# GSByeon/multi-speaker-tacotron-tensorflow

Measured on AMD Instinct MI355X. Metric: mel-frames/sec (batched decode), higher is better.
Workload: dtype f32 storage and accumulation; feed-forward GEMMs as 3-term split-bf16 MFMA (bf16x3), the attention memory layer as 6-term split-bf16 MFMA (operands split three ways: fp32-grade); recurrent / decoder mat-vecs exact fp32

## Files before the change

### include/taco_debug.h

```cpp
#ifndef TACO_DEBUG_H
#define TACO_DEBUG_H

#include "taco_abi.h"

#ifdef __cplusplus
extern "C" {
#endif

int taco_debug_set_persistent(taco_model* m, int on);

int taco_debug_set_bf3(taco_model* m, int on, int tile_n);

int taco_debug_set_fuse_prenet(taco_model* m, int on);
int taco_debug_set_fuse_concat(taco_model* m, int on);
int taco_debug_set_att_split(taco_model* m, int slices);
int taco_debug_set_overlap(taco_model* m, int on);

int taco_debug_set_decoder_persist(taco_model* m, int mode, int rows_per_group);
int taco_debug_raise_device_error(taco_model* m, int value);
int taco_debug_decoder_info(taco_model* m, int* out16);
int taco_debug_decoder_trace(taco_model* m, int enable, long long* out);

int taco_debug_set_skip_scans(taco_model* m, int on);

int taco_debug_set_chip_turns(int on);

int taco_debug_force_gemm_config(taco_model* m, int cfg);

int taco_debug_set_front(taco_model* m, int delay_clocks, int prio);

int taco_train_debug_bigru(taco_train* t, void* hip_stream, const float* d_xproj, const int32_t* d_lengths, const float* d_h0,
                           const float* d_dout, int B, int T, int persistent, float* d_out, float* d_gsave, float* d_dg, float* d_rh,
                           float* d_dh0, void* d_scratch, size_t scratch_bytes);

int taco_debug_wgrad_plan(int wgrad_bf3, int wgrad_planes, int deterministic, long long det_floats, long long planes_uint4, int region_open,
                          int M, int T, int K, int N, int kw, int padl, int gather, int ygather, int nw, int* out8);

int taco_debug_spec_epilogue(taco_gl* g, void* hip_stream, const float* d_est, int R, float* d_linear, float* d_mel);

int taco_debug_gl_create_host(const taco_audio_hparams* hp, int tf_flavor, taco_gl** out);

#ifdef __cplusplus
}
#endif
#endif
```

### multi-speaker-tacotron-tensorflow_amd/_lib.py

```python
import ctypes as C
import os

from .hparams import MODEL_TYPES, ATTENTION_TYPES, NUM_SYMBOLS

_HERE = os.path.dirname(os.path.abspath(__file__))
LIB_PATH = os.path.join(_HERE, "csrc", "libtaco_hip.so")

TACO_ERR_ARG, TACO_ERR_SHAPE, TACO_ERR_UNSUPPORTED, TACO_ERR_HIP, TACO_ERR_STATE = -1, -2, -3, -4, -5
TACO_TRIM_SPECTRAL, TACO_TRIM_TIME = 0, 1
TACO_WAV_F32, TACO_WAV_PCM16 = 0, 1


class TacoHParams(C.Structure):
    _fields_ = [
        ("num_symbols", C.c_int32), ("num_mels", C.c_int32), ("num_freq", C.c_int32),
        ("num_speakers", C.c_int32), ("model_type", C.c_int32), ("speaker_embedding_size", C.c_int32),
        ("embedding_size", C.c_int32),
        ("enc_prenet_n", C.c_int32), ("enc_prenet", C.c_int32 * 4),
        ("enc_bank_size", C.c_int32), ("enc_bank_channels", C.c_int32), ("enc_maxpool", C.c_int32),
        ("enc_highway_depth", C.c_int32), ("enc_rnn_size", C.c_int32),
        ("enc_proj_n", C.c_int32), ("enc_proj", C.c_int32 * 4), ("enc_proj_width", C.c_int32),
        ("attention_type", C.c_int32), ("attention_size", C.c_int32), ("attention_state_size", C.c_int32),
        ("dec_layer_num", C.c_int32), ("dec_rnn_size", C.c_int32),
        ("dec_prenet_n", C.c_int32), ("dec_prenet", C.c_int32 * 4),
# ... 13 lines not shown
class TacoCollateStream(C.Structure):
    _fields_ = [("pack", C.c_void_p), ("start", C.c_void_p), ("rows", C.c_void_p), ("width", C.c_int32), ("rows_out", C.c_int32),
                ("out", C.c_void_p), ("counts", C.c_void_p)]


TACO_COLLATE_MAX_STREAMS = 8


class TacoError(Exception):

    def __init__(self, code, msg):
        super().__init__(msg)
        self.code = code


def _list4(vals, what):
    vals = list(vals)
    if not 1 <= len(vals) <= 4:
        raise TacoError(TACO_ERR_ARG, "%s must have 1..4 entries, got %d" % (what, len(vals)))
    arr = (C.c_int32 * 4)(*(vals + [0] * (4 - len(vals))))
    return len(vals), arr


def to_c_hparams(hp, num_speakers):
    if hp.model_type not in MODEL_TYPES:
        raise Exception(" [!] Unkown multi-speaker model type: {}".format(hp.model_type))
    if hp.attention_type not in ATTENTION_TYPES:
        raise Exception(" [!] Unkown attention type: {}".format(hp.attention_type))
    c = TacoHParams()
    c.num_symbols = getattr(hp, "num_symbols", NUM_SYMBOLS)
    c.num_mels, c.num_freq = hp.num_mels, hp.num_freq
    c.num_speakers = int(num_speakers)
    c.model_type = MODEL_TYPES[hp.model_type]
    c.speaker_embedding_size = hp.speaker_embedding_size
    c.embedding_size = hp.embedding_size
    c.enc_prenet_n, c.enc_prenet = _list4(hp.enc_prenet_sizes, "enc_prenet_sizes")
    c.enc_bank_size, c.enc_bank_channels = hp.enc_bank_size, hp.enc_bank_channel_size
    c.enc_maxpool, c.enc_highway_depth, c.enc_rnn_size = hp.enc_maxpool_width, hp.enc_highway_depth, hp.enc_rnn_size
    c.enc_proj_n, c.enc_proj = _list4(hp.enc_proj_sizes, "enc_proj_sizes")
    c.enc_proj_width = hp.enc_proj_width
    c.attention_type = ATTENTION_TYPES[hp.attention_type]
    c.attention_size, c.attention_state_size = hp.attention_size, hp.attention_state_size
    c.dec_layer_num, c.dec_rnn_size = hp.dec_layer_num, hp.dec_rnn_size
    c.dec_prenet_n, c.dec_prenet = _list4(hp.dec_prenet_sizes, "dec_prenet_sizes")
    c.post_bank_size, c.post_bank_channels = hp.post_bank_size, hp.post_bank_channel_size
    c.post_maxpool, c.post_highway_depth, c.post_rnn_size = hp.post_maxpool_width, hp.post_highway_depth, hp.post_rnn_size
    c.post_proj_n, c.post_proj = _list4(hp.post_proj_sizes, "post_proj_sizes")
    c.post_proj_width = hp.post_proj_width
    c.reduction_factor, c.max_iters = hp.reduction_factor, hp.max_iters
    return c


_P = C.c_void_p
_I = C.c_int
_S = C.c_size_t
SYNC_SUM_FN = C.CFUNCTYPE(None, C.c_void_p, C.c_void_p, C.c_int)

PROTOTYPES = {
    "taco_abi_version": (_I, []),
    "taco_last_error": (C.c_char_p, []),
    "taco_model_create": (_I, [C.POINTER(TacoHParams), _I, C.POINTER(_P)]),
    "taco_model_set_weight": (_I, [_P, C.c_char_p, _P, C.POINTER(C.c_int64), _I]),
    "taco_model_num_weights": (_I, [_P]),
    "taco_model_weight_name": (_I, [_P, _I, C.c_char_p, _I, C.POINTER(C.c_int64), C.POINTER(_I)]),
    "taco_model_finalize": (_I, [_P]),
    "taco_model_destroy": (None, [_P]),
    "taco_workspace_bytes": (_S, [_P, _I, _I, _I]),
    "taco_stage_workspace_bytes": (_S, [_P, _I, _I]),
    "taco_forward_infer": (_I, [_P, _P, _P, _P, _P, _I, _I, _I, _P, _P, _P, _P, _P, _P, _S]),
    "taco_plan_create": (_I, [_P, _P, _P, _P, _I, _I, _I, _P, _P, _P, _P, _P, _P, _S, C.POINTER(_P)]),
    "taco_plan_launch": (_I, [_P, _P]),
    "taco_plan_num_nodes": (_I, [_P]),
    "taco_plan_whole_chip": (_I, [_P]),
    "taco_plan_destroy": (None, [_P]),
    "taco_encoder_forward": (_I, [_P, _P, _P, _P, _P, _I, _I, _P, _P, _S]),
    "taco_decoder_forward": (_I, [_P, _P, _P, _P, _I, _I, _I, _P, _P, _P, _P, _P, _P, _P, _S]),
    "taco_postnet_forward": (_I, [_P, _P, _P, _P, _I, _I, _P, _P, _P, _S]),
    "taco_conv1d_bn_f32": (_I, [_P, _P, C.c_char_p, _P, _I, _I, _I, _I, _P]),
    "taco_dense_f32": (_I, [_P, _P, C.c_char_p, _P, _I, _I, _P]),
    "taco_highway_f32": (_I, [_P, _P, C.c_char_p, _P, _I, _P]),
    "taco_bigru_f32": (_I, [_P, _P, C.c_char_p, _P, _P, _P, _I, _I, _P, _P, _S]),
    "taco_attention_step_f32": (_I, [_P, _P, _P, _P, _P, _P, _I, _I, _P, _P, _P, _S]),
    "taco_gru_cell_f32": (_I, [_P, _P, C.c_char_p, _P, _P, _I, _P, _P, _S]),
    "taco_gl_create": (_I, [C.POINTER(TacoAudioHParams), _I, C.POINTER(_P)]),
    "taco_gl_destroy": (None, [_P]),
    "taco_gl_num_samples": (_I, [_P, _I]),
    "taco_gl_workspace_bytes": (_S, [_P, _I, _I]),
    "taco_gl_inv_spectrogram": (_I, [_P, _P, _P, _P, C.c_ulonglong, _I, _I, _I, _P, _P, _S]),
    "taco_gl_min_frames": (_I, [_P]),
    "taco_gl_rows_workspace_bytes": (_S, [_P, _I, _I]),
    "taco_gl_inv_spectrogram_rows": (_I, [_P, _P, _P, _P, _P, C.c_ulonglong, _I, _I, _I, _P, _P, _P, _S]),
    "taco_wav_to_pcm16": (_I, [_P, _P, _P, _I, _I, _P]),
    "taco_gl_create_tf": (_I, [C.POINTER(TacoAudioHParams), _I, C.POINTER(_P)]),
    "taco_gl_tf_num_samples": (_I, [_P, _I]),
    "taco_gl_tf_workspace_bytes": (_S, [_P, _I, _I]),
    "taco_gl_inv_spectrogram_tf": (_I, [_P, _P, _P, _P, _I, _I, _I, _P, _P, _P, _S]),
    "taco_gl_set_inv_mel_basis": (_I, [_P, _P, _I]),
    "taco_gl_mel_to_linear": (_I, [_P, _P, _P, _I, _I, _P]),
    "taco_gl_inv_melspectrogram_rows": (_I, [_P, _P, _P, _P, _P, C.c_ulonglong, _I, _I, _I, _P, _P, _P, _S]),
    "taco_debug_gl_create_host": (_I, [C.POINTER(TacoAudioHParams), _I, C.POINTER(_P)]),
    "taco_wav_trim_workspace_bytes": (_S, [_I, _I, _I, _I]),
    "taco_wav_trim": (_I, [_P, _P, _P, _I, _I, C.c_float, _I, _I, _I, _P, _P, _P, _S]),
    "taco_wav_split_workspace_bytes": (_S, [_I, _I, _I, _I]),
    "taco_wav_split": (_I, [_P, _P, _P, _I, _I, C.c_float, _I, _I, _I, _I, _P, _P, _P, _P, _S]),
    "taco_wav_breath_mute": (_I, [_P, _P, _P, _I, _I, _P, _P, _I, C.c_float, _P, _P, _P]),
    "taco_resample_create": (_I, [_I, _I, _P, _I, _I, _I, C.POINTER(_P)]),
    "taco_resample_destroy": (None, [_P]),
    "taco_resample_out_len": (_I, [_P, _I]),
    "taco_resample_computed_len": (_I, [_P, _I]),
    "taco_resample_phases": (_I, [_P]),
    "taco_resample_taps": (_I, [_P]),
    "taco_resample_left_taps": (_I, [_P]),
    "taco_resample_tile": (_I, [_P]),
    "taco_resample_bank": (_I, [_P, _P]),
    "taco_wav_resample": (_I, [_P, _P, _P, _I, _I, _P, _I, _I, _P, _I, _P]),
    "taco_gl_set_mel_basis": (_I, [_P, _P, _I]),
    "taco_spec_num_mels": (_I, [_P]),
    "taco_spec_num_frames": (_I, [C.POINTER(TacoAudioHParams), _I]),
    "taco_spec_workspace_bytes": (_S, [_P, _I, _I]),
    "taco_spec_targets": (_I, [_P, _P, _P, _P, _I, _I, _P, _P, _P, _P, _S]),
    "taco_collate": (_I, [_P, C.POINTER(TacoCollateStream), _I, _P, _I, _I]),
    "taco_debug_spec_epilogue": (_I, [_P, _P, _P, _I, _P, _P]),
    "taco_attention_trim": (_I, [_P, _P, _P, _I, _I, _I, _I, _P]),
    "taco_loss_f32": (_I, [_P, _P, _P, _P, _P, _P, _I, _I, _I, _I, _I, _I, _P, _P, _S]),
    "taco_learning_rate": (C.c_float, [C.c_longlong, C.c_float, _I, _I]),
    "taco_adam_step_f32": (_I, [_P, _P, _P, _P, _P, _S, C.c_longlong, C.c_float, C.c_float, C.c_float, C.c_float, C.c_float, _P, _P, _S]),
    "taco_train_create": (_I, [C.POINTER(TacoHParams), _I, C.POINTER(_P)]),
    "taco_train_destroy": (None, [_P]),
    "taco_train_model": (_P, [_P]),
    "taco_train_num_params": (_S, [_P]),
    "taco_train_param_offset": (_I, [_P, C.c_char_p, C.POINTER(_S)]),
    "taco_train_refresh": (_I, [_P, _P, _P]),
    "taco_train_set_sync_bn": (_I, [_P, _P, _P, _I]),
    "taco_train_set_deterministic": (_I, [_P, _I]),
    "taco_train_set_exact_wgrad": (_I, [_P, _I]),
    "taco_train_set_wgrad_planes": (_I, [_P, _I]),
    "taco_train_planes_problems": (_I, [_P]),
    "taco_train_set_bptt_engine": (_I, [_P, _I]),
    "taco_train_set_exact_gemm": (_I, [_P, _I]),
    "taco_debug_wgrad_plan": (_I, [_I, _I, _I, C.c_longlong, C.c_longlong, _I, _I, _I, _I, _I, _I, _I, _I, _I, _I, C.POINTER(_I)]),
    "taco_train_debug_bigru": (_I, [_P, _P, _P, _P, _P, _P, _I, _I, _I, _P, _P, _P, _P, _P, _P, _S]),
    "taco_train_workspace_bytes": (_S, [_P, _I, _I, _I]),
    "taco_train_forward_backward": (_I, [_P, _P, _P, _P, _P, _P, _P, _P, _P, _P, _I, _I, _I, _I, _I, _P, _P, _P, _P, _I, _P, _S]),
    "taco_debug_force_gemm_config": (_I, [_P, _I]),
    "taco_debug_set_skip_scans": (_I, [_P, _I]),
    "taco_debug_set_chip_turns": (_I, [_I]),
    "taco_debug_set_front": (_I, [_P, _I, _I]),
    "taco_debug_set_persistent": (_I, [_P, _I]),
    "taco_debug_set_overlap": (_I, [_P, _I]),
    "taco_stop_steps": (_I, [_P, _P, _I, _I, _I, _I, _P]),
    "taco_debug_set_fuse_prenet": (_I, [_P, _I]),
    "taco_debug_set_fuse_concat": (_I, [_P, _I]),
    "taco_debug_set_att_split": (_I, [_P, _I]),
    "taco_debug_set_bf3": (_I, [_P, _I, _I]),
    "taco_model_device_errors": (_I, [_P, C.POINTER(_I)]),
    "taco_debug_raise_device_error": (_I, [_P, _I]),
    "taco_debug_set_decoder_persist": (_I, [_P, _I, _I]),
    "taco_debug_decoder_info": (_I, [_P, C.POINTER(_I)]),
    "taco_model_engine_plan": (_I, [_P, _I, _I, _I, _I, C.c_char_p, _I]),
    "taco_model_set_batch_invariant": (_I, [_P, _I]),
    "taco_debug_decoder_trace": (_I, [_P, _I, C.POINTER(C.c_longlong)]),
}

_lib = None


def load_library(path=None):
    global _lib
    if _lib is not None and path is None:
        return _lib
    p = path or os.environ.get("TACO_LIB") or LIB_PATH
    if path is None and os.environ.get("TACO_LIB") and os.path.abspath(p) != os.path.abspath(LIB_PATH):
        import warnings
        warnings.warn("TACO_LIB overrides the library: loading %s instead of %s" % (p, LIB_PATH), RuntimeWarning, stacklevel=2)
    if not os.path.exists(p):
        raise ImportError(
            "libtaco_hip.so not found at %s -- build it first (python -c 'import __graft_entry__ as g; g.build()' "
            "or multi-speaker-tacotron-tensorflow_amd/csrc/build.sh).  There is no CPU fallback." % p)
    lib = C.CDLL(p)
    for name, (res, args) in PROTOTYPES.items():
        fn = getattr(lib, name)
        fn.restype = res
        fn.argtypes = args
    if lib.taco_abi_version() != 1:
        raise ImportError("libtaco_hip.so ABI version %d, expected 1" % lib.taco_abi_version())
    if path is None:
        _lib = lib
    return lib


def check(rc):
    if rc != 0:
        msg = load_library().taco_last_error().decode("utf-8", "replace")
        if rc == TACO_ERR_UNSUPPORTED and msg.startswith(" [!]"):
            raise Exception(msg)
        raise TacoError(rc, "libtaco_hip error %d: %s" % (rc, msg))
```

### multi-speaker-tacotron-tensorflow_amd/csrc/taco_chain.h

```cpp
#pragma once
#include "taco_kernels.h"

#define CH_MAXL 8
#ifndef CH_PF256
#define CH_PF256 2
#endif
#ifndef CH_PF128
#define CH_PF128 2
#endif
#ifndef CH_ROT
#define CH_ROT 1
#endif
#define CH_BM 64
enum { CH_DENSE = 0, CH_HIGHWAY = 1, CH_XPROJ = 2 };
struct ChainLayer {
  const unsigned short* bh; const unsigned short* bl; const unsigned short* bh2; const unsigned short* bl2;
  const float* bias; const float* bias2;
  int type, K16, NT, N, act;
};
struct ChainEntry {
  const float* part; int P; size_t MN; int N1;
  const float* b1; const float* s1; const float* h1; int relu1;
  const unsigned short* bh; const unsigned short* bl; int NT2, K16tap, N2;
  const float* b2; const float* s2; const float* h2;
  const float* res; int ldres;
  const float* rowvec; int ldrv;
};
struct ChainArgs {
  ChainEntry e;
  const float* x; int ldx, Cin;
  const int* gather;
  float* out; int ldo;
  float* y; int ldy;
  const int* rev_len; int rev_col0;
  int M, T, nlayers;
  int krot;
  int ntiles; unsigned* zp[4]; unsigned long long znw[4];
  ChainLayer L[CH_MAXL];
};

template <int TM, int LDSW, bool DUAL, int CH_PF>
__device__ __forceinline__ void ch_mma_loop(int K16, int NT, const unsigned short* bhA, const unsigned short* blA, int nt,
                                            const unsigned short* bhB, const unsigned short* blB, int nt2,
                                            const unsigned short* xhi, const unsigned short* xlo, int row0,
                                            int l31, int lh, f32x16 (&acc)[TM], f32x16 (&acc2)[TM], int rot = 0) {
  auto kstep = [&](int g) { const int gg = min(g, K16 - 1) + rot; return gg >= K16 ? gg - K16 : gg; };
  auto boff = [&](int g, int t) { return ((((size_t)kstep(g) * NT + t) * 2 + lh) * 32 + l31) * 8; };
  uint4 ph, pl, ph2, pl2, qh, ql, qh2, ql2;
  ph2 = pl2 = qh2 = ql2 = make_uint4(0, 0, 0, 0);
  auto loadb = [&](int g, uint4& h, uint4& l, uint4& h2, uint4& l2) {
    const size_t o = boff(g, nt);
    h = *reinterpret_cast<const uint4*>(bhA + o); l = *reinterpret_cast<const uint4*>(blA + o);
    if constexpr (DUAL) { const size_t o2 = boff(g, nt2); h2 = *reinterpret_cast<const uint4*>(bhB + o2); l2 = *reinterpret_cast<const uint4*>(blB + o2); }
  };
  auto mma = [&](int g, const uint4& h, const uint4& l, const uint4& h2, const uint4& l2) {
    const bf16x8 bh = __builtin_bit_cast(bf16x8, h), bl = __builtin_bit_cast(bf16x8, l);
    bf16x8 ah[TM], al[TM];
#pragma unroll
    for (int tm = 0; tm < TM; ++tm) {
      const int off = (row0 + tm * 32 + l31) * LDSW + 16 * kstep(g) + 8 * lh;
      ah[tm] = __builtin_bit_cast(bf16x8, *reinterpret_cast<const uint4*>(xhi + off));
      al[tm] = __builtin_bit_cast(bf16x8, *reinterpret_cast<const uint4*>(xlo + off));
    }
#pragma unroll
    for (int tm = 0; tm < TM; ++tm) acc[tm] = __builtin_amdgcn_mfma_f32_32x32x16_bf16(al[tm], bh, acc[tm], 0, 0, 0);
#pragma unroll
    for (int tm = 0; tm < TM; ++tm) acc[tm] = __builtin_amdgcn_mfma_f32_32x32x16_bf16(ah[tm], bl, acc[tm], 0, 0, 0);
#pragma unroll
    for (int tm = 0; tm < TM; ++tm) acc[tm] = __builtin_amdgcn_mfma_f32_32x32x16_bf16(ah[tm], bh, acc[tm], 0, 0, 0);
    if constexpr (DUAL) {
      const bf16x8 bh2 = __builtin_bit_cast(bf16x8, h2), bl2 = __builtin_bit_cast(bf16x8, l2);
#pragma unroll
      for (int tm = 0; tm < TM; ++tm) acc2[tm] = __builtin_amdgcn_mfma_f32_32x32x16_bf16(al[tm], bh2, acc2[tm], 0, 0, 0);
#pragma unroll
      for (int tm = 0; tm < TM; ++tm) acc2[tm] = __builtin_amdgcn_mfma_f32_32x32x16_bf16(ah[tm], bl2, acc2[tm], 0, 0, 0);
#pragma unroll
      for (int tm = 0; tm < TM; ++tm) acc2[tm] = __builtin_amdgcn_mfma_f32_32x32x16_bf16(ah[tm], bh2, acc2[tm], 0, 0, 0);
    }
  };
  if constexpr (CH_PF == 2) {
  loadb(0, ph, pl, ph2, pl2);
  for (int g = 0; g < K16; g += 2) {
    loadb(g + 1, qh, ql, qh2, ql2);
    __builtin_amdgcn_sched_barrier(0);
    mma(g, ph, pl, ph2, pl2);
    __builtin_amdgcn_sched_barrier(0);
    loadb(g + 2, ph, pl, ph2, pl2);
    __builtin_amdgcn_sched_barrier(0);
    mma(g + 1, qh, ql, qh2, ql2);
    __builtin_amdgcn_sched_barrier(0);
  }
  } else {
  uint4 rh[CH_PF], rl[CH_PF], rh2[CH_PF], rl2[CH_PF];
#pragma unroll
  for (int i = 0; i < CH_PF; ++i) rh2[i] = rl2[i] = make_uint4(0, 0, 0, 0);
#pragma unroll
  for (int i = 0; i < CH_PF - 1; ++i) loadb(i, rh[i], rl[i], rh2[i], rl2[i]);
  for (int g = 0; g < K16; g += CH_PF) {
#pragma unroll
    for (int i = 0; i < CH_PF; ++i) {
      loadb(g + i + CH_PF - 1, rh[(i + CH_PF - 1) % CH_PF], rl[(i + CH_PF - 1) % CH_PF], rh2[(i + CH_PF - 1) % CH_PF], rl2[(i + CH_PF - 1) % CH_PF]);
      __builtin_amdgcn_sched_barrier(0);
      if (g + i < K16) mma(g + i, rh[i], rl[i], rh2[i], rl2[i]);
      __builtin_amdgcn_sched_barrier(0);
    }
  }
  }
}

#ifdef TACO_TRACE
__device__ long long taco_trace_chain[64];
#define CTRC(i) do { if (trc && (i) < 64) taco_trace_chain[i] = clock64(); } while (0)
#else
#define CTRC(i) do {} while (0)
#endif
template <int W>
__global__ __launch_bounds__(512) void k_pointwise_chain(const ChainArgs a_in) {
  constexpr int WN = W / 32, WM = 8 / WN, TM = CH_BM / 32 / WM;
  constexpr int PF = W == 256 ? CH_PF256 : CH_PF128;
  constexpr int LDSW = W + 8;
  extern __shared__ __attribute__((aligned(16))) unsigned short ch_smem[];
  unsigned short* xhi = ch_smem;
  unsigned short* xlo = ch_smem + CH_BM * LDSW;
  struct { const float* x; float* out; float* y; const int* rev_len; int ldx, Cin, ldo, ldy, rev_col0, M, T, nlayers; } a =
      {a_in.x, a_in.out, a_in.y, a_in.rev_len, a_in.ldx, a_in.Cin, a_in.ldo, a_in.ldy, a_in.rev_col0, a_in.M, a_in.T, a_in.nlayers};
  PIN(a.x); PIN(a.out); PIN(a.y); PIN(a.rev_len); PIN(a.ldx); PIN(a.Cin); PIN(a.ldo); PIN(a.ldy); PIN(a.rev_col0); PIN(a.M); PIN(a.T);
  PIN(a.nlayers);
  const int tid = threadIdx.x, lane = tid & 63, l31 = lane & 31, lh = lane >> 5;
  const int wave = __builtin_amdgcn_readfirstlane(tid >> 6);
  const int wm = wave / WN, wn = wave % WN;
  if (a_in.ntiles > 0 && (int)blockIdx.x >= a_in.ntiles) {
    const size_t i0 = (size_t)((int)blockIdx.x - a_in.ntiles) * 512 + tid, stride = (size_t)((int)gridDim.x - a_in.ntiles) * 512;
    for (int rg = 0; rg < 4; ++rg) {
      unsigned* p = a_in.zp[rg];
      const size_t nw = a_in.znw[rg];
      if (!p || !nw) continue;
      const size_t n16 = (reinterpret_cast<uintptr_t>(p) & 15) ? 0 : nw / 4;
      uint4* q = reinterpret_cast<uint4*>(p);
      for (size_t i = i0; i < n16; i += stride) q[i] = make_uint4(0u, 0u, 0u, 0u);
      for (size_t i = n16 * 4 + i0; i < nw; i += stride) p[i] = 0u;
    }
    return;
  }
  const int m0 = blockIdx.x * CH_BM;
  const int krot = (CH_ROT && a_in.krot) ? ((int)(blockIdx.x >> 3) & 31) : 0;
#ifdef TACO_TRACE
  const bool trc = (blockIdx.x == (a_in.ntiles > 0 ? a_in.ntiles : gridDim.x) / 2) && threadIdx.x == 0;
  int trci = 5;
  CTRC(0);
#endif

  const int l31_outer = l31, lh_outer = lh;
  float xreg[TM][16];
  bool have_x = false;
  if (a_in.e.part) {
    const ChainEntry E = a_in.e;
    const float* gpart = E.part; const float* gb1 = E.b1; const float* gs1 = E.s1; const float* gh1 = E.h1;
    const unsigned short* gbh = E.bh; const unsigned short* gbl = E.bl;
    const float* gres = E.res; const float* grv = E.rowvec; const float* gb2 = E.b2; const float* gs2 = E.s2; const float* gh2 = E.h2;
    PIN(gpart); PIN(gb1); PIN(gs1); PIN(gh1); PIN(gbh); PIN(gbl); PIN(gres); PIN(grv); PIN(gb2); PIN(gs2); PIN(gh2);
    const int LDE = E.N1 + 8;
    unsigned short* ehi = ch_smem + 2 * CH_BM * LDSW;
    unsigned short* elo = ehi + (CH_BM + 2) * LDE;
    const int nq = E.N1 / 4;
    constexpr int NSTG = ((CH_BM + 2) * (256 / 4) + 511) / 512;
    {
      float4 f[NSTG];
      const float* src[NSTG];
#pragma unroll
      for (int u = 0; u < NSTG; ++u) {
        const int i = tid + 512 * u, r = i / nq, c = 4 * (i - r * nq), row = m0 - 1 + r;
        f[u] = make_float4(0.f, 0.f, 0.f, 0.f);
        src[u] = (i < (CH_BM + 2) * nq && row >= 0 && row < a.M) ? gpart + (size_t)row * E.N1 + c : nullptr;
      }
      int q = 0;
      for (; q + 1 < E.P; q += 2) {
        float4 g[NSTG], g2[NSTG];
#pragma unroll
        for (int u = 0; u < NSTG; ++u) {
          g[u] = src[u] ? *reinterpret_cast<const float4*>(src[u] + (size_t)q * E.MN) : make_float4(0.f, 0.f, 0.f, 0.f);
          g2[u] = src[u] ? *reinterpret_cast<const float4*>(src[u] + (size_t)(q + 1) * E.MN) : make_float4(0.f, 0.f, 0.f, 0.f);
        }
#pragma unroll
        for (int u = 0; u < NSTG; ++u) { f[u].x += g[u].x; f[u].y += g[u].y; f[u].z += g[u].z; f[u].w += g[u].w; }
#pragma unroll
        for (int u = 0; u < NSTG; ++u) { f[u].x += g2[u].x; f[u].y += g2[u].y; f[u].z += g2[u].z; f[u].w += g2[u].w; }
      }
      if (q < E.P) {
        float4 g[NSTG];
#pragma unroll
        for (int u = 0; u < NSTG; ++u) g[u] = src[u] ? *reinterpret_cast<const float4*>(src[u] + (size_t)q * E.MN) : make_float4(0.f, 0.f, 0.f, 0.f);
#pragma unroll
        for (int u = 0; u < NSTG; ++u) { f[u].x += g[u].x; f[u].y += g[u].y; f[u].z += g[u].z; f[u].w += g[u].w; }
      }
#pragma unroll
      for (int u = 0; u < NSTG; ++u) {
        const int i = tid + 512 * u, r = i / nq, c = 4 * (i - r * nq);
        if (i >= (CH_BM + 2) * nq) continue;
        float4 v = f[u];
        if (src[u]) {
          const float4 bi = gb1 ? *reinterpret_cast<const float4*>(gb1 + c) : make_float4(0.f, 0.f, 0.f, 0.f);
          const float4 sc = gs1 ? *reinterpret_cast<const float4*>(gs1 + c) : make_float4(1.f, 1.f, 1.f, 1.f);
          const float4 sh = gh1 ? *reinterpret_cast<const float4*>(gh1 + c) : make_float4(0.f, 0.f, 0.f, 0.f);
          v.x += bi.x; v.y += bi.y; v.z += bi.z; v.w += bi.w;
          if (E.relu1) { v.x = fmaxf(v.x, 0.f); v.y = fmaxf(v.y, 0.f); v.z = fmaxf(v.z, 0.f); v.w = fmaxf(v.w, 0.f); }
          v.x = v.x * sc.x + sh.x; v.y = v.y * sc.y + sh.y; v.z = v.z * sc.z + sh.z; v.w = v.w * sc.w + sh.w;
        }
        uint2 h4, l4;
        taco_split_bf16x4(v, h4, l4);
        *reinterpret_cast<uint2*>(ehi + r * LDE + c) = h4;
        *reinterpret_cast<uint2*>(elo + r * LDE + c) = l4;
      }
    }
    CTRC(1);
    __syncthreads();
    const int K0 = a_in.L[0].K16 * 16;
    const int col = wn * 32 + l31;
    const bool cin = col < E.N2;
    float rs[TM][16];
#pragma unroll
    for (int tm = 0; tm < TM; ++tm)
#pragma unroll
      for (int r = 0; r < 16; ++r) {
        const int rl = (wm * TM + tm) * 32 + (r & 3) + 8 * (r >> 2) + 4 * lh, row = min(m0 + rl, a.M - 1);
        float v = 0.f;
        if (cin) {
          v = gres[(size_t)row * E.ldres + col];
          if (grv) v += grv[(size_t)(row / a.T) * E.ldrv + col];
        }
        rs[tm][r] = v;
      }
    f32x16 acc[TM];
#pragma unroll
    for (int tm = 0; tm < TM; ++tm)
      for (int r = 0; r < 16; ++r) acc[tm][r] = 0.f;
    const int KSPL = (WM == 1 && 2 * E.NT2 <= WN) ? 2 : 1;
    const bool mact = wn < E.NT2 * KSPL;
    const int ect = mact ? wn % E.NT2 : 0, kp = mact ? wn / E.NT2 : 0;
    if (mact) {
      int tloc[TM];
#pragma unroll
      for (int tm = 0; tm < TM; ++tm) tloc[tm] = (m0 + (wm * TM + tm) * 32 + l31) % a.T;
      const int nk = (3 * E.K16tap) / KSPL, kbeg = kp * nk, kend = kbeg + nk;
      auto boff = [&](int k) { return ((((size_t)k * E.NT2 + ect) * 2 + lh) * 32 + l31) * 8; };
      constexpr int NB = 6;
      uint4 pH[NB], pL[NB], qH[NB], qL[NB];
      auto loadblk = [&](int k0, uint4 (&H)[NB], uint4 (&Lo)[NB]) {
#pragma unroll
        for (int i = 0; i < NB; ++i) { const size_t o = boff(min(k0 + i, kend - 1)); H[i] = *reinterpret_cast<const uint4*>(gbh + o); Lo[i] = *reinterpret_cast<const uint4*>(gbl + o); }
      };
      auto mmablk = [&](int k0, const uint4 (&H)[NB], const uint4 (&Lo)[NB]) {
#pragma unroll
        for (int i = 0; i < NB; ++i) {
          const int k = k0 + i, j = k / E.K16tap, g = k - j * E.K16tap;
          const bf16x8 bh8 = __builtin_bit_cast(bf16x8, H[i]), bl8 = __builtin_bit_cast(bf16x8, Lo[i]);
#pragma unroll
          for (int tm = 0; tm < TM; ++tm) {
            const int off = ((wm * TM + tm) * 32 + l31 + j) * LDE + 16 * g + 8 * lh;
            uint4 xh = *reinterpret_cast<const uint4*>(ehi + off), xl = *reinterpret_cast<const uint4*>(elo + off);
            const int tt = tloc[tm] + j - 1;
            const unsigned keep = ((tt >= 0) && (tt < a.T)) ? 0xffffffffu : 0u;
            xh.x &= keep; xh.y &= keep; xh.z &= keep; xh.w &= keep; xl.x &= keep; xl.y &= keep; xl.z &= keep; xl.w &= keep;
            const bf16x8 ah = __builtin_bit_cast(bf16x8, xh), al = __builtin_bit_cast(bf16x8, xl);
            acc[tm] = __builtin_amdgcn_mfma_f32_32x32x16_bf16(al, bh8, acc[tm], 0, 0, 0);
            acc[tm] = __builtin_amdgcn_mfma_f32_32x32x16_bf16(ah, bl8, acc[tm], 0, 0, 0);
            acc[tm] = __builtin_amdgcn_mfma_f32_32x32x16_bf16(ah, bh8, acc[tm], 0, 0, 0);
          }
        }
      };
      loadblk(kbeg, pH, pL);
      for (int k0 = kbeg; k0 < kend; k0 += 2 * NB) {
        loadblk(k0 + NB, qH, qL);
        __builtin_amdgcn_sched_barrier(0);
        mmablk(k0, pH, pL);
        __builtin_amdgcn_sched_barrier(0);
        loadblk(k0 + 2 * NB, pH, pL);
        __builtin_amdgcn_sched_barrier(0);
        mmablk(k0 + NB, qH, qL);
        __builtin_amdgcn_sched_barrier(0);
      }
    }
    if (KSPL == 2) {
      float* red = reinterpret_cast<float*>(ch_smem);
      if (mact && kp == 1) {
#pragma unroll
        for (int tm = 0; tm < TM; ++tm)
#pragma unroll
          for (int r = 0; r < 16; ++r) red[((ect * TM + tm) * 16 + r) * 64 + lane] = acc[tm][r];
      }
      __syncthreads();
      if (mact && kp == 0) {
#pragma unroll
        for (int tm = 0; tm < TM; ++tm)
#pragma unroll
          for (int r = 0; r < 16; ++r) acc[tm][r] += red[((ect * TM + tm) * 16 + r) * 64 + lane];
      } else {
#pragma unroll
        for (int tm = 0; tm < TM; ++tm)
          for (int r = 0; r < 16; ++r) acc[tm][r] = 0.f;
      }
      __syncthreads();
    }
    CTRC(2);
    {
      const float bi = (cin && gb2) ? gb2[col] : 0.f, sc = (cin && gs2) ? gs2[col] : 1.f, sh = (cin && gh2) ? gh2[col] : 0.f;
#pragma unroll
      for (int tm = 0; tm < TM; ++tm)
#pragma unroll
        for (int r = 0; r < 16; ++r) asm volatile("" : "+v"(rs[tm][r]));
#pragma unroll
      for (int tm = 0; tm < TM; ++tm)
#pragma unroll
        for (int r = 0; r < 16; ++r) {
          const int rl = (wm * TM + tm) * 32 + (r & 3) + 8 * (r >> 2) + 4 * lh;
          const float v = cin ? (acc[tm][r] + bi) * sc + sh + rs[tm][r] : 0.f;
          xreg[tm][r] = v;
          if (col < K0) {
            const unsigned hp = taco_pk_bf16(v, 0.f) & 0xffffu;
            const unsigned lp = taco_pk_bf16(v - __uint_as_float(hp << 16), 0.f) & 0xffffu;
            xhi[rl * LDSW + col] = (unsigned short)hp;
            xlo[rl * LDSW + col] = (unsigned short)lp;
          }
        }
      have_x = true;
    }
    CTRC(3);
  } else
  {
    const int K0 = a_in.L[0].K16 * 16;
    for (int i = tid; i < CH_BM * (K0 / 4); i += 512) {
      const int r = i / (K0 / 4), c = 4 * (i % (K0 / 4));
      float4 f = make_float4(0.f, 0.f, 0.f, 0.f);
      const int row = m0 + r;
      if (row < a.M && c < a.Cin) {
        const float* p = a.x + (size_t)(a_in.gather ? a_in.gather[row] : row) * a.ldx + c;
        if (c + 3 < a.Cin && (a.ldx & 3) == 0) f = *reinterpret_cast<const float4*>(p);
        else { f.x = p[0]; if (c + 1 < a.Cin) f.y = p[1]; if (c + 2 < a.Cin) f.z = p[2]; if (c + 3 < a.Cin) f.w = p[3]; }
      }
      uint2 h4, l4;
      taco_split_bf16x4(f, h4, l4);
      *reinterpret_cast<uint2*>(xhi + r * LDSW + c) = h4;
      *reinterpret_cast<uint2*>(xlo + r * LDSW + c) = l4;
    }
  }
  const bool full = m0 + CH_BM <= a.M;
  __syncthreads();
  CTRC(4);

  for (int li = 0; li < a.nlayers; ++li) {
    const ChainLayer L = a_in.L[li];
    int l31 = l31_outer, lh = lh_outer;
    asm volatile("" : "+v"(l31), "+v"(lh));
    auto rloc = [&](int tm, int r) { return (wm * TM + tm) * 32 + (r & 3) + 8 * (r >> 2) + 4 * lh; };
    const int col = wn * 32 + l31;
    if (L.type == CH_XPROJ) {
      const int ngroups = (L.N + W - 1) / W;
      const int bb0 = m0 / a.T;
      const int nbrow = (a.M - 1) / a.T;
      const int Lb0 = a.rev_len ? a.rev_len[min(bb0, nbrow)] : a.T, Lb1 = a.rev_len ? a.rev_len[min(bb0 + 1, nbrow)] : a.T;
      auto store_group = [&](int ng, const f32x16 (&acc)[TM]) {
        const int ocol = ng * W + col;
        if (ocol >= L.N) return;
        const float bia = L.bias ? L.bias[ocol] : 0.f;
        const bool rev = a.rev_col0 >= 0 && ocol >= a.rev_col0;
        const bool relu_out = L.act == ACT_RELU;
        if (full && !rev) {
#pragma unroll
          for (int tm = 0; tm < TM; ++tm) {
            float* po = a.out + (size_t)(m0 + rloc(tm, 0)) * a.ldo + ocol;
#pragma unroll
            for (int r = 0; r < 16; ++r) { const float v = acc[tm][r] + bia; po[(size_t)((r & 3) + 8 * (r >> 2)) * a.ldo] = relu_out ? fmaxf(v, 0.f) : v; }
          }
        } else {
          int lhs = lh;
          asm volatile("" : "+v"(lhs));
#pragma unroll
          for (int tm = 0; tm < TM; ++tm)
#pragma unroll
            for (int r = 0; r < 16; ++r) {
              const int row = m0 + (wm * TM + tm) * 32 + (r & 3) + 8 * (r >> 2) + 4 * lhs;
              int orow = row;
              if (rev) {
                const int bb = a.T >= CH_BM ? bb0 + (row >= (bb0 + 1) * a.T ? 1 : 0) : row / a.T;
                const int tt = row - bb * a.T, Lb = a.T >= CH_BM ? (bb == bb0 ? Lb0 : Lb1) : (a.rev_len ? a.rev_len[min(bb, (a.M - 1) / a.T)] : a.T);
                orow = tt < Lb ? bb * a.T + (Lb - 1 - tt) : row;
              }
              if (row < a.M) { const float v = acc[tm][r] + bia; a.out[(size_t)orow * a.ldo + ocol] = relu_out ? fmaxf(v, 0.f) : v; }
            }
        }
      };
      const int npass = (ngroups + 1) / 2, odd = ngroups & 1;
      for (int ps = 0; ps < npass; ++ps) {
        const int ng = (odd && ps == 0) ? ngroups - 1 : 2 * (ps - odd);
        const int nt = min(ng * WN + wn, L.NT - 1), nt2 = min((ng + 1) * WN + wn, L.NT - 1);
        f32x16 acc[TM], acc2[TM];
#pragma unroll
        for (int tm = 0; tm < TM; ++tm)
          for (int r = 0; r < 16; ++r) { acc[tm][r] = 0.f; acc2[tm][r] = 0.f; }
        if (ng + 1 < ngroups) ch_mma_loop<TM, LDSW, true, PF>(L.K16, L.NT, L.bh, L.bl, nt, L.bh, L.bl, nt2, xhi, xlo, wm * TM * 32, l31, lh, acc, acc2, krot * L.K16 >> 5);
        else ch_mma_loop<TM, LDSW, false, PF>(L.K16, L.NT, L.bh, L.bl, nt, L.bh, L.bl, nt, xhi, xlo, wm * TM * 32, l31, lh, acc, acc2, krot * L.K16 >> 5);
#ifdef TACO_TRACE
        CTRC(trci); ++trci;
#endif
        store_group(ng, acc);
        if (ng + 1 < ngroups) store_group(ng + 1, acc2);
#ifdef TACO_TRACE
        CTRC(trci); ++trci;
#endif
      }
      continue;
    }
    const bool dual = L.type == CH_HIGHWAY;
    if (dual && !have_x) {
#pragma unroll
      for (int tm = 0; tm < TM; ++tm)
#pragma unroll
        for (int r = 0; r < 16; ++r) xreg[tm][r] = a.x[(size_t)min(m0 + rloc(tm, r), a.M - 1) * a.ldx + col];
    }
    have_x = true;
    {
      f32x16 acc[TM], acc2[TM];
#pragma unroll
      for (int tm = 0; tm < TM; ++tm)
        for (int r = 0; r < 16; ++r) { acc[tm][r] = 0.f; acc2[tm][r] = 0.f; }
      const float bia = L.bias ? L.bias[col] : 0.f;
      if (dual) {
        const float bia2 = L.bias2 ? L.bias2[col] : 0.f;
        ch_mma_loop<TM, LDSW, true, PF>(L.K16, L.NT, L.bh, L.bl, wn, L.bh2, L.bl2, wn, xhi, xlo, wm * TM * 32, l31, lh, acc, acc2, krot * L.K16 >> 5);
#ifdef TACO_TRACE
        CTRC(trci); ++trci;
#endif
#pragma unroll
        for (int tm = 0; tm < TM; ++tm)
#pragma unroll
          for (int r = 0; r < 16; ++r) {
            const float Hh = fmaxf(acc[tm][r] + bia, 0.f);
            const float Tg = __builtin_amdgcn_rcpf(1.0f + __builtin_amdgcn_exp2f(-1.4426950408889634f * (acc2[tm][r] + bia2)));
            xreg[tm][r] = Hh * Tg + xreg[tm][r] * (1.f - Tg);
          }
      } else {
        ch_mma_loop<TM, LDSW, false, PF>(L.K16, L.NT, L.bh, L.bl, wn, L.bh, L.bl, wn, xhi, xlo, wm * TM * 32, l31, lh, acc, acc2, krot * L.K16 >> 5);
#ifdef TACO_TRACE
        CTRC(trci); ++trci;
#endif
        const bool relu = L.act == ACT_RELU;
#pragma unroll
        for (int tm = 0; tm < TM; ++tm)
#pragma unroll
          for (int r = 0; r < 16; ++r) { const float v = acc[tm][r] + bia; xreg[tm][r] = relu ? fmaxf(v, 0.f) : v; }
      }
    }
    const bool last_hidden = (li + 1 == a.nlayers) || a_in.L[li + 1].type == CH_XPROJ;
    if (last_hidden && a.y) {
#pragma unroll
      for (int tm = 0; tm < TM; ++tm)
#pragma unroll
        for (int r = 0; r < 16; ++r) {
          const int row = m0 + rloc(tm, r);
          if (row < a.M) a.y[(size_t)row * a.ldy + col] = xreg[tm][r];
        }
    }
#ifdef TACO_TRACE
    CTRC(trci); ++trci;
#endif
    __syncthreads();
#ifdef TACO_TRACE
    CTRC(trci); ++trci;
#endif
#pragma unroll
    for (int tm = 0; tm < TM; ++tm)
#pragma unroll
      for (int r = 0; r < 16; ++r) {
        const float f = xreg[tm][r];
        const unsigned hp = taco_pk_bf16(f, 0.f) & 0xffffu;
        const unsigned lp = taco_pk_bf16(f - __uint_as_float(hp << 16), 0.f) & 0xffffu;
        xhi[rloc(tm, r) * LDSW + col] = (unsigned short)hp;
        xlo[rloc(tm, r) * LDSW + col] = (unsigned short)lp;
      }
    __syncthreads();
#ifdef TACO_TRACE
    CTRC(trci); ++trci;
#endif
  }
}
```

### multi-speaker-tacotron-tensorflow_amd/csrc/taco_lib.hip

```cpp
#include "taco_kernels.h"
#include "taco_decoder_xcd.h"
#include "taco_bigru_xcd.h"
#include "taco_chain.h"
#include "taco_front.h"
#include "taco_head.h"
#include "taco_train_kernels.h"
#include "taco_backward_kernels.h"
#include "taco_wgrad_planes.h"
#include "taco_decoder_bwd_xcd.h"
#include "../../include/taco_abi.h"
#include "../../include/taco_debug.h"

#include <algorithm>
#include <cmath>
#include <cstdarg>
#include <cstdio>
#include <cstring>
#include <cstdlib>
#include <functional>
#include <map>
#include <string>
#include <vector>

static thread_local std::string g_err;
// ... 42 lines not shown
  for (size_t i = n16 * 4 + i0; i < nw; i += stride) p[i] = 0u;
}
struct ZeroRegions { uint32_t* p[4]; unsigned long long nw[4]; };
__global__ void k_zero_fill_multi(const ZeroRegions z) {
  uint32_t* p = z.p[blockIdx.y];
  const size_t nw = z.nw[blockIdx.y];
  const size_t n16 = (reinterpret_cast<uintptr_t>(p) & 15) ? 0 : nw / 4;
  const size_t i0 = (size_t)blockIdx.x * blockDim.x + threadIdx.x, stride = (size_t)gridDim.x * blockDim.x;
  uint4* q = reinterpret_cast<uint4*>(p);
  for (size_t i = i0; i < n16; i += stride) q[i] = make_uint4(0u, 0u, 0u, 0u);
  for (size_t i = n16 * 4 + i0; i < nw; i += stride) p[i] = 0u;
}
#define ZM_MAX 12
struct ZeroMany { uint32_t* p[ZM_MAX]; unsigned long long nw[ZM_MAX]; };
__global__ void k_zero_fill_many(const ZeroMany z) {
  uint32_t* p = z.p[blockIdx.y];
  const size_t nw = z.nw[blockIdx.y];
  const size_t n16 = (reinterpret_cast<uintptr_t>(p) & 15) ? 0 : nw / 4;
  const size_t i0 = (size_t)blockIdx.x * blockDim.x + threadIdx.x, stride = (size_t)gridDim.x * blockDim.x;
  uint4* q = reinterpret_cast<uint4*>(p);
  for (size_t i = i0; i < n16; i += stride) q[i] = make_uint4(0u, 0u, 0u, 0u);
  for (size_t i = n16 * 4 + i0; i < nw; i += stride) p[i] = 0u;
}
struct ClearedSet { const void* p[8]; size_t n[8]; int cnt; };
static thread_local ClearedSet g_cleared = {};
static void register_cleared(const ZeroRegions& z) {
  for (int i = 0; i < 4; ++i)
    if (z.p[i] && g_cleared.cnt < 8) { g_cleared.p[g_cleared.cnt] = z.p[i]; g_cleared.n[g_cleared.cnt++] = z.nw[i] * 4; }
}
static hipError_t zero_async(void* p, size_t bytes, hipStream_t st);
static hipError_t clear_polled(void* p, size_t bytes, hipStream_t st) {
  for (int i = 0; i < g_cleared.cnt; ++i)
    if (g_cleared.p[i] == p && g_cleared.n[i] >= bytes) return hipSuccess;
  return zero_async(p, bytes, st);
}
static hipError_t zero_async(void* p, size_t bytes, hipStream_t st) {
  if (!bytes) return hipSuccess;
  if ((reinterpret_cast<uintptr_t>(p) & 3) || (bytes & 3)) return hipMemsetAsync(p, 0, bytes, st);
  const size_t nw = bytes / 4;
  const size_t n16 = (reinterpret_cast<uintptr_t>(p) & 15) ? 0 : nw / 4;
  const size_t items = n16 ? n16 + (nw - n16 * 4) : nw;
  const unsigned blocks = (unsigned)std::min<size_t>((items + 255) / 256, 2048);
  hipLaunchKernelGGL(k_zero_fill, dim3(blocks), dim3(256), 0, st, static_cast<uint32_t*>(p), n16, nw);
  return hipGetLastError();
}

struct ZeroBatch {
  ZeroMany z; int n = 0; size_t big = 0; hipStream_t st;
  explicit ZeroBatch(hipStream_t s) : st(s) { memset(&z, 0, sizeof z); }
  hipError_t add(void* p, size_t bytes) {
    if (!bytes) return hipSuccess;
    if ((reinterpret_cast<uintptr_t>(p) & 3) || (bytes & 3)) return zero_async(p, bytes, st);
    if (n == ZM_MAX) { hipError_t e = run(); if (e != hipSuccess) return e; }
    z.p[n] = static_cast<uint32_t*>(p); z.nw[n] = bytes / 4; big = std::max(big, bytes / 16); ++n;
    return hipSuccess;
  }
  hipError_t run() {
    if (!n) return hipSuccess;
    const unsigned blocks = (unsigned)std::min<size_t>(std::max<size_t>((big + 255) / 256, 1), 1024);
    hipLaunchKernelGGL(k_zero_fill_many, dim3(blocks, n), dim3(256), 0, st, z);
    n = 0; big = 0; memset(&z, 0, sizeof z);
    return hipGetLastError();
  }
};

#define HIPCHK(expr)                                                                        \
  do {                                                                                      \
    hipError_t e_ = (expr);                                                                 \
    if (e_ != hipSuccess) return fail(TACO_ERR_HIP, "%s: %s", #expr, hipGetErrorString(e_)); \
  } while (0)
#define TRY(expr)            \
  do {                       \
    int rc_ = (expr);        \
    if (rc_ != 0) return rc_; \
  } while (0)

static inline int cdiv(int a, int b) { return (a + b - 1) / b; }
static inline int rup(int a, int b) { return cdiv(a, b) * b; }
static inline size_t rup_sz(size_t a, size_t b) { return (a + b - 1) / b * b; }

struct HostTensor {
  std::vector<int64_t> shape;
  std::vector<float> data;
  bool set = false;
};

struct ConvL {
  int kw = 1, cin = 0, cin_pad = 0, N = 0;
  size_t wp = 0, wp2 = 0, bias = 0, bias2 = 0, bns = 0, bnb = 0;
  size_t bh = 0, bl = 0, bh2 = 0, bl2 = 0;
  size_t bl3 = 0, bl3_2 = 0;
  bool x6 = false;
  int K16 = 0, cin_pad16 = 0;
  size_t wtail = 0; int ntail = 0;
  int var_index = -1;
};
struct SkW {
  int K = 0, Kq = 0, N = 0;
  size_t wp = 0, bias = 0;
};
struct GruDec { SkW gx, ch; int I = 0, H = 0; };
struct Cbhg {
  int in_dim = 0, K = 0, C = 0, maxpool = 1, depth = 0, rnn = 0, pw = 3;
  int nproj = 0, proj_dim[4] = {0, 0, 0, 0};
  std::vector<ConvL> bank;
  int bank_var0 = -1;
  std::vector<ConvL> proj;
  bool has_dense = false;
  ConvL dense;
  std::vector<ConvL> hw;
  ConvL xproj;
  SkW gh[2], ch[2];
  size_t raw_gh[2] = {0, 0}, raw_ch[2] = {0, 0};
  size_t res_g2[2] = {0, 0};
  size_t gd_pack = 0, gb_pack = 0;
  size_t gob_pack = 0;
  size_t go_pack[3] = {0, 0, 0};
  std::vector<size_t> fr_wh, fr_wl; std::vector<int> fr_ns; int front_kind = 0;
  size_t res_g2p[2] = {0, 0}, res_c1p[2] = {0, 0};
};

struct taco_model {
  taco_hparams hp;
  int device = 0;
  bool finalized = false;
  std::vector<std::pair<std::string, std::vector<int64_t>>> spec;
  std::map<std::string, HostTensor> raw;
  std::vector<float> harena;
  float* darena = nullptr;
  size_t arena_n = 0;
  std::vector<GemmVar> hvars;
  std::map<std::string, ConvL> convs;
  std::map<std::string, SkW> skinny;
  std::map<std::string, GruDec> grus;
  std::vector<ConvL> enc_prenet;
  Cbhg enc, post;
  ConvL memory_layer, linear;
  std::vector<SkW> dec_prenet;
  GruDec att_gru;
  std::vector<GruDec> dec_gru;
  SkW query, concat_proj, frame_proj, lin_spk;
  SkW prenet1_next;
  int fuse_prenet1 = 1;
  GruDec gru1_fold;
  int fuse_concat = 0;
  int att_split = -1;
  size_t att_v = 0, att_b = 0, att_sb = 0, emb = 0, spk_emb = 0, raw_wq = 0;
  std::vector<SkW> spk_dense;
  std::vector<size_t> spk_table;
  int force_cfg = -1;
  unsigned* d_err = nullptr;
  int persist = 1;
  int ff_rot = 1;
  int bf3 = 1;
  int bf3x6 = 0;
  int bf3_tn = 0;
  int chain = 1;
  int front_entry = 1;
  int front_prio = 1; int front_delay = 0;
  int head_sweep = 1;
  int front = 1;
  int overlap = 0;
  size_t dx_fold_n = 0;
  size_t dx_spkw = 0;
  std::vector<unsigned> bf3_idx; std::vector<Bf3Seg> bf3_segs;
  int last_bptt = 0;
  size_t dbx_pack = 0;
  size_t dx_pack = 0, dx_p1o_raw = 0, dx_qpack[4] = {0, 0, 0, 0}, dx_b_p1_0 = 0, dx_b_p1c = 0, dx_b_p2 = 0, dx_b_p3 = 0, dx_b_ag = 0, dx_b_ac = 0, dx_b_g1f = 0,
         dx_b_g1c = 0, dx_b_g2g = 0, dx_b_g2c = 0, dx_b_f = 0;
  int cu_count = 0;
  int dx_mode = 1;
  int dx_rows = 0;
  long long* d_trace = nullptr;
  int trace_on = 0;
  int skip_scans = 0;
  hipStream_t side = nullptr;
  std::vector<hipEvent_t> events;
  struct TrainPacks* tp = nullptr;
};
static int build_train_packs(taco_model* m);

static size_t arena_put(taco_model* m, const float* src, size_t n) {
  size_t off = rup_sz(m->harena.size(), 16);
  m->harena.resize(off + rup_sz(std::max<size_t>(n, 1), 16), 0.f);
  if (src) memcpy(&m->harena[off], src, n * sizeof(float));
  return off + 1;
}
static inline const float* AP(const taco_model* m, size_t off1) { return off1 ? m->darena + (off1 - 1) : nullptr; }

static void spec_add(taco_model* m, const std::string& n, std::vector<int64_t> s) { m->spec.push_back({n, s}); }
static void spec_dense(taco_model* m, const std::string& n, int i, int o, bool bias = true) {
  spec_add(m, n + "/kernel", {i, o});
  if (bias) spec_add(m, n + "/bias", {o});
}
static void spec_conv(taco_model* m, const std::string& n, int k, int i, int o) {
  spec_add(m, n + "/kernel", {k, i, o});
  spec_add(m, n + "/bias", {o});
  for (const char* p : {"gamma", "beta", "moving_mean", "moving_variance"}) spec_add(m, n + "/" + p, {o});
}
static void spec_gru(taco_model* m, const std::string& n, int i, int h) {
  spec_add(m, n + "/gates/kernel", {i + h, 2 * h});
  spec_add(m, n + "/gates/bias", {2 * h});
  spec_add(m, n + "/candidate/kernel", {i + h, h});
  spec_add(m, n + "/candidate/bias", {h});
}
static void spec_cbhg(taco_model* m, const std::string& sc, int in_dim, int K, int C, int depth, int rnn,
                      const int* projs, int nproj, int pw) {
  for (int k = 1; k <= K; ++k) spec_conv(m, sc + "/conv_bank/conv1d_" + std::to_string(k), k, in_dim, C);
  int d = K * C;
  for (int i = 0; i < nproj; ++i) {
    spec_conv(m, sc + "/proj_" + std::to_string(i + 1), pw, d, projs[i]);
    d = projs[i];
  }
  if (d != rnn) spec_dense(m, sc + "/dense", d, rnn);
  for (int i = 0; i < depth; ++i) {
    spec_dense(m, sc + "/highway_" + std::to_string(i + 1) + "/H", rnn, rnn);
    spec_dense(m, sc + "/highway_" + std::to_string(i + 1) + "/T", rnn, rnn);
  }
  spec_gru(m, sc + "/bigru/fw", rnn, rnn);
  spec_gru(m, sc + "/bigru/bw", rnn, rnn);
}
static const char* kSpkNames[3] = {"before_highway", "encoder_rnn_init", "attention_rnn_init"};

static int build_spec(taco_model* m) {
  const taco_hparams& hp = m->hp;
  m->spec.clear();
  spec_add(m, "embedding", {hp.num_symbols, hp.embedding_size});
  const bool multi = hp.num_speakers > 1;
  const int spk = hp.speaker_embedding_size;
  if (multi) {
    if (spk != 1) spec_add(m, "speaker_embedding", {hp.num_speakers, spk});
    if (hp.model_type == 2) {
      std::vector<std::pair<std::string, int>> dims = {{kSpkNames[0], hp.enc_prenet[hp.enc_prenet_n - 1]},
                                                       {kSpkNames[1], hp.enc_rnn_size * 2},
                                                       {kSpkNames[2], hp.attention_state_size}};
      for (int i = 0; i < hp.dec_layer_num; ++i) dims.push_back({"decoder_rnn_init_" + std::to_string(i + 1), hp.dec_rnn_size});
      for (auto& d : dims) {
        if (spk == 1) spec_add(m, "spk/" + d.first + "/table", {hp.num_speakers, d.second});
        else spec_dense(m, "spk/" + d.first, spk, d.second);
      }
    }
  }
  int d = hp.embedding_size;
  for (int i = 0; i < hp.enc_prenet_n; ++i) {
    spec_dense(m, "prenet/dense_" + std::to_string(i + 1), d, hp.enc_prenet[i]);
    d = hp.enc_prenet[i];
  }
  spec_cbhg(m, "encoder_cbhg", d, hp.enc_bank_size, hp.enc_bank_channels, hp.enc_highway_depth, hp.enc_rnn_size,
            hp.enc_proj, hp.enc_proj_n, hp.enc_proj_width);
  const int enc_out = 2 * hp.enc_rnn_size, A = hp.attention_size;
  spec_dense(m, "attention/memory_layer", enc_out, A, false);
  spec_dense(m, "attention/query_layer", hp.attention_state_size, A, false);
  spec_add(m, "attention/attention_v", {A});
  if (hp.attention_type == 2) spec_add(m, "attention/attention_score_bias", {});
  if (hp.attention_type == 1) {
    spec_add(m, "attention/attention_g", {});
    spec_add(m, "attention/attention_b", {A});
  }
  d = hp.num_mels + enc_out;
  for (int i = 0; i < hp.dec_prenet_n; ++i) {
    spec_dense(m, "decoder/prenet/dense_" + std::to_string(i + 1), d, hp.dec_prenet[i]);
    d = hp.dec_prenet[i];
  }
  const int sspk = (multi && hp.model_type == 1) ? spk : 0;
  spec_gru(m, "decoder/attention_gru", d + sspk, hp.attention_state_size);
  spec_dense(m, "decoder/concat_projection", hp.attention_state_size + enc_out + sspk, hp.dec_rnn_size);
  for (int i = 0; i < hp.dec_layer_num; ++i) spec_gru(m, "decoder/gru_" + std::to_string(i + 1), hp.dec_rnn_size, hp.dec_rnn_size);
  spec_dense(m, "decoder/frame_projection", hp.dec_rnn_size, hp.num_mels * hp.reduction_factor);
  spec_cbhg(m, "post_cbhg", hp.num_mels, hp.post_bank_size, hp.post_bank_channels, hp.post_highway_depth,
            hp.post_rnn_size, hp.post_proj, hp.post_proj_n, hp.post_proj_width);
  spec_dense(m, "linear", 2 * hp.post_rnn_size + sspk, hp.num_freq);
  return 0;
}

static size_t pack_w32(taco_model* m, const float* W, int kw, int cin, int N, int* cin_pad_out, int* Kq_out, int* NT_out) {
  const int cin_pad = rup(cin, 8), Kq = kw * cin_pad / 4, NT = cdiv(N, 32);
  std::vector<float> p((size_t)NT * Kq * 32 * 4, 0.f);
  for (int nt = 0; nt < NT; ++nt)
    for (int kq = 0; kq < Kq; ++kq)
      for (int j = 0; j < 32; ++j)
        for (int e = 0; e < 4; ++e) {
          const int k = 4 * kq + e, tap = k / cin_pad, c = k % cin_pad, n = 32 * nt + j;
          if (c < cin && n < N) p[(((size_t)nt * Kq + kq) * 32 + j) * 4 + e] = W[((size_t)tap * cin + c) * N + n];
        }
  *cin_pad_out = cin_pad; *Kq_out = Kq; *NT_out = NT;
  return arena_put(m, p.data(), p.size());
}
static unsigned short bf16_rne_host(float x) {
  unsigned u; memcpy(&u, &x, 4);
  return (unsigned short)((u + 0x7FFFu + ((u >> 16) & 1u)) >> 16);
}
static void pack_bf3(taco_model* m, const float* W, int kw, int cin, int N, size_t* hi_out, size_t* lo_out, int* K16_out, int* cp16_out, size_t* l3_out = nullptr) {
  const int cp16 = rup(cin, 32), K16 = kw * cp16 / 16, NT = cdiv(N, 32);
  std::vector<unsigned short> hi((size_t)NT * K16 * 2 * 32 * 8, 0), lo(hi.size(), 0);
  std::vector<unsigned> idx(m->tp ? hi.size() : 0, 0u);
  const bool want_l3 = l3_out && !m->tp && *l3_out == (size_t)1;
  std::vector<unsigned short> l3v(want_l3 ? hi.size() : 0, 0);
  for (int nt = 0; nt < NT; ++nt)
    for (int k16 = 0; k16 < K16; ++k16)
      for (int h = 0; h < 2; ++h)
        for (int j = 0; j < 32; ++j)
          for (int e = 0; e < 8; ++e) {
            const int k = 16 * k16 + 8 * h + e, tap = k / cp16, c = k % cp16, n = 32 * nt + j;
            if (c < cin && n < N) {
              const float w = W[((size_t)tap * cin + c) * N + n];
              const size_t oi = ((((size_t)k16 * NT + nt) * 2 + h) * 32 + j) * 8 + e;
// ... 781 lines not shown
  HIPCHK(hipMemcpyToSymbol(HIP_SYMBOL(g_go_knob), d, sizeof d));
#endif
  return 0;
}
template <bool TAPE, bool TRACE>
static void duo_launch_rg(int RG, dim3 grid, dim3 blk, size_t lds, hipStream_t st, const GdArgs& a) {
  switch (RG) {
    case 1: hipLaunchKernelGGL((k_bigru_duo<1, TAPE, TRACE>), grid, blk, lds, st, a); break;
    case 2: hipLaunchKernelGGL((k_bigru_duo<2, TAPE, TRACE>), grid, blk, lds, st, a); break;
    case 4: hipLaunchKernelGGL((k_bigru_duo<4, TAPE, TRACE>), grid, blk, lds, st, a); break;
    default: hipLaunchKernelGGL((k_bigru_duo<8, TAPE, TRACE>), grid, blk, lds, st, a); break;
  }
}
template <bool TAPE, bool TRACE>
static void oct_launch_upw(int UPW, dim3 grid, dim3 blk, size_t lds, hipStream_t st, const GdArgs& a) {
  switch (UPW) {
    case 1: hipLaunchKernelGGL((k_bigru_oct<1, TAPE, TRACE>), grid, blk, lds, st, a); break;
    case 2: hipLaunchKernelGGL((k_bigru_oct<2, TAPE, TRACE>), grid, blk, lds, st, a); break;
    default: hipLaunchKernelGGL((k_bigru_oct<4, TAPE, TRACE>), grid, blk, lds, st, a); break;
  }
}
static int duo_launch(const taco_model* m, hipStream_t st, const Cbhg& c, int RG, int B, int T, const float* xproj, const int* lengths, const float* init_state,
                      float* out, float* gsave, unsigned long long* gxbuf, unsigned* gxctl) {
  ChipTurn turn(m->device, st);
  GdArgs a; memset(&a, 0, sizeof a);
  a.wpack = AP(m, c.gd_pack); a.xproj = xproj; a.h0 = init_state; a.lengths = lengths; a.out = out; a.gsave = gsave;
  a.xbuf = gxbuf; a.ctl = gxctl; a.err = m->d_err; a.trace = (m->trace_on && m->d_trace && !gsave) ? m->d_trace + DX_TRACE_STEPS * DX_TRACE_SLOTS : nullptr;
  a.B = B; a.T = T; a.force_wt = m->dx_mode == 2 ? 1 : 0;
  HIPCHK(clear_polled(gxbuf, (size_t)((char*)gxctl - (char*)gxbuf) + 256, st));
  const size_t lds = std::max(gd_lds_floats(RG) * sizeof(float), (size_t)96 * 1024);
  const dim3 grid(DX_NGROUP * GD_MEMBERS), blk(512);
  if (a.trace) duo_launch_rg<false, true>(RG, grid, blk, lds, st, a);
  else if (gsave) duo_launch_rg<true, false>(RG, grid, blk, lds, st, a);
  else duo_launch_rg<false, false>(RG, grid, blk, lds, st, a);
  HIPCHK(hipGetLastError());
  return 0;
}
static int duo_bwd_launch(const taco_model* m, hipStream_t st, const Cbhg& c, int RG, int B, int T, const float* dout, const float* out, const float* gsave,
                          const float* h0, const int* lengths, float* dg, float* rh, float* dh0, unsigned long long* gxbuf, unsigned* gxctl) {
  ChipTurn turn(m->device, st);
  GbArgs a; memset(&a, 0, sizeof a);
  a.wpack = AP(m, c.gb_pack); a.dout = dout; a.out = out; a.gsave = gsave; a.h0 = h0; a.lengths = lengths; a.dg = dg; a.rh = rh; a.dh0 = dh0;
  a.xbuf = gxbuf; a.ctl = gxctl; a.err = m->d_err; a.B = B; a.T = T; a.force_wt = m->dx_mode == 2 ? 1 : 0;
  const size_t lds = std::max(gb_lds_floats(RG) * sizeof(float), (size_t)96 * 1024);
  const dim3 grid(DX_NGROUP * GD_MEMBERS), blk(512);
  switch (RG) {
    case 1: hipLaunchKernelGGL((k_bigru_duo_bwd<1>), grid, blk, lds, st, a); break;
    case 2: hipLaunchKernelGGL((k_bigru_duo_bwd<2>), grid, blk, lds, st, a); break;
    case 4: hipLaunchKernelGGL((k_bigru_duo_bwd<4>), grid, blk, lds, st, a); break;
    default: hipLaunchKernelGGL((k_bigru_duo_bwd<8>), grid, blk, lds, st, a); break;
  }
  HIPCHK(hipGetLastError());
  return 0;
}
static int oct_bwd_launch(const taco_model* m, hipStream_t st, const Cbhg& c, int B, int T, const float* dout, const float* out, const float* gsave,
                          const float* h0, const int* lengths, float* dg, float* rh, float* dh0, unsigned long long* gxbuf, unsigned* gxctl) {
  ChipTurn turn(m->device, st);
  TRY(go_knob_upload());
  GbArgs a; memset(&a, 0, sizeof a);
  a.wpack = AP(m, c.gob_pack); a.dout = dout; a.out = out; a.gsave = gsave; a.h0 = h0; a.lengths = lengths; a.dg = dg; a.rh = rh; a.dh0 = dh0;
  a.xbuf = gxbuf; a.ctl = gxctl; a.err = m->d_err; a.B = B; a.T = T; a.force_wt = m->dx_mode == 2 ? 1 : 0;
  const size_t lds = std::max(gob_lds_floats() * sizeof(float), (size_t)96 * 1024);
  hipLaunchKernelGGL(k_bigru_oct_bwd, dim3(CHIP_CUS), dim3(512), lds, st, a);
  HIPCHK(hipGetLastError());
  return 0;
}
static int oct_launch(const taco_model* m, hipStream_t st, const Cbhg& c, int UPW, int B, int T, const float* xproj, const int* lengths, const float* init_state,
                      float* out, float* gsave, unsigned long long* gxbuf, unsigned* gxctl) {
  ChipTurn turn(m->device, st);
  TRY(go_knob_upload());
  GdArgs a; memset(&a, 0, sizeof a);
  a.wpack = AP(m, c.go_pack[UPW == 4 ? 2 : UPW == 2 ? 1 : 0]); a.xproj = xproj; a.h0 = init_state; a.lengths = lengths; a.out = out; a.gsave = gsave;
  a.xbuf = gxbuf; a.ctl = gxctl; a.err = m->d_err; a.trace = (m->trace_on && m->d_trace && !gsave) ? m->d_trace + DX_TRACE_STEPS * DX_TRACE_SLOTS : nullptr;
  a.B = B; a.T = T; a.force_wt = m->dx_mode == 2 ? 1 : 0;
  HIPCHK(clear_polled(gxbuf, (size_t)((char*)gxctl - (char*)gxbuf) + 256, st));
  const size_t lds = std::max(go_lds_floats(UPW) * sizeof(float), (size_t)96 * 1024);
  const dim3 grid(CHIP_CUS), blk(512);
  if (a.trace) oct_launch_upw<false, true>(UPW, grid, blk, lds, st, a);
  else if (gsave) oct_launch_upw<true, false>(UPW, grid, blk, lds, st, a);
  else oct_launch_upw<false, false>(UPW, grid, blk, lds, st, a);
  HIPCHK(hipGetLastError());
  return 0;
}

static int bigru_scan(const taco_model* m, hipStream_t st, const Cbhg& c, int B, int T,
                      const int* lengths, const float* init_state, float* out, const CbhgWs& w) {
  const int H = c.rnn;
  if (m->skip_scans) return 0;
  const ScanPlan sp = scan_plan(m, c, B, T);
  if (sp.kernel == SCAN_K_OCT) return oct_launch(m, st, c, sp.upw, B, T, w.xproj, lengths, init_state, out, nullptr, w.gxbuf, w.gxctl);
  if (sp.kernel == SCAN_K_DUO) return duo_launch(m, st, c, sp.rg, B, T, w.xproj, lengths, init_state, out, nullptr, w.gxbuf, w.gxctl);
  if (sp.kernel == SCAN_K_RESW || sp.kernel == SCAN_K_RES || sp.kernel == SCAN_K_QUAD) {
    BigruSArgs a; memset(&a, 0, sizeof a);
    a.xproj = w.xproj; a.g2_0 = (const float2*)AP(m, c.res_g2[0]); a.g2_1 = (const float2*)AP(m, c.res_g2[1]);
    a.c1_0 = AP(m, c.raw_ch[0]); a.c1_1 = AP(m, c.raw_ch[1]); a.h0 = init_state; a.lengths = lengths; a.out = out; a.B = B; a.T = T;
    const dim3 grid(2 * B);
    if (sp.kernel == SCAN_K_RESW) {
      a.g2_0 = (const float2*)AP(m, c.res_g2p[0]); a.g2_1 = (const float2*)AP(m, c.res_g2p[1]); a.c1_0 = AP(m, c.res_c1p[0]); a.c1_1 = AP(m, c.res_c1p[1]);
      const size_t lds = ((size_t)3 * H + (size_t)8 * 3 * H) * sizeof(float) + (size_t)4 * 8 * H * 12;
      hipLaunchKernelGGL((k_bigru_resw<16, 4, 2>), grid, dim3(512), lds, st, a);
    }
    else if (sp.kernel == SCAN_K_QUAD) hipLaunchKernelGGL(k_bigru_quad<false>, grid, dim3(512), 0, st, a);
    else if (H == 256) hipLaunchKernelGGL((k_bigru_res<256, 64, 24, 1, false>), grid, dim3(512), bigru_res_lds(256, 24, 1), st, a);
    else hipLaunchKernelGGL((k_bigru_res<128, 32, 0, 1, false>), grid, dim3(512), bigru_res_lds(128, 0, 1), st, a);
    HIPCHK(hipGetLastError());
    return 0;
  }
  if (sp.kernel == SCAN_K_ROWS) {
    int R = 0; size_t lds = 0;
    bigru_rows_cfg(B, H, &R, &lds);
    BigruRArgs a; memset(&a, 0, sizeof a);
    a.xproj = w.xproj; a.wg0 = AP(m, c.raw_gh[0]); a.wg1 = AP(m, c.raw_gh[1]); a.wc0 = AP(m, c.raw_ch[0]); a.wc1 = AP(m, c.raw_ch[1]);
    a.h0 = init_state; a.lengths = lengths; a.out = out; a.B = B; a.T = T; a.H = H;
    const dim3 grid(2 * cdiv(B, R));
    if (R == 2) hipLaunchKernelGGL((k_bigru_rows<2, false>), grid, dim3(RP_NT), lds, st, a);
    else hipLaunchKernelGGL((k_bigru_rows<1, false>), grid, dim3(RP_NT), lds, st, a);
    HIPCHK(hipGetLastError());
    return 0;
  }
  for (int dir = 0; dir < 2; ++dir)
    hipLaunchKernelGGL(k_copy2d, dim3(cdiv(B * H, 256)), dim3(256), 0, st, init_state ? init_state + dir * H : nullptr,
                       2 * H, w.h + (size_t)dir * B * H, H, B, H);
  HIPCHK(hipGetLastError());
  for (int s = 0; s < T; ++s) {
    SkJob ja[2], jb[2];
    for (int dir = 0; dir < 2; ++dir) {
      float* h = w.h + (size_t)dir * B * H; float* rh = w.rh + (size_t)dir * B * H; float* u = w.u + (size_t)dir * B * H;
      ja[dir] = sk_base(m, c.gh[dir], h, H, H, nullptr, 0);
      ja[dir].H = H; ja[dir].e0 = h; ja[dir].lde0 = H;
      ja[dir].e1 = w.xproj + dir * 3 * H; ja[dir].lde1 = 6 * H;
      ja[dir].o0 = rh; ja[dir].ldo0 = H; ja[dir].o1 = u; ja[dir].ldo1 = H;
      ja[dir].step = s; ja[dir].T = T; ja[dir].dir = dir;
      jb[dir] = sk_base(m, c.ch[dir], rh, H, H, nullptr, 0);
      jb[dir].H = H; jb[dir].e0 = h; jb[dir].lde0 = H;
      jb[dir].e1 = w.xproj + dir * 3 * H + 2 * H; jb[dir].lde1 = 6 * H; jb[dir].e2 = u; jb[dir].lde2 = H;
      jb[dir].o0 = h; jb[dir].ldo0 = H; jb[dir].o2 = out; jb[dir].ldo2 = 2 * H; jb[dir].seq_coff = dir * H;
      jb[dir].lengths = lengths; jb[dir].step = s; jb[dir].T = T; jb[dir].dir = dir;
    }
    TRY(run_skinny(st, B, ja, 2, EPI_GRU_GATES));
    TRY(run_skinny(st, B, jb, 2, EPI_GRU_CAND));
  }
  return 0;
}

static bool chain_fits(const Cbhg& c, int in_dim) {
  const int W = c.rnn;
  if (W != 128 && W != 256) return false;
  if ((int)c.hw.size() != c.depth || c.depth + (c.has_dense ? 2 : 1) > CH_MAXL) return false;
  if (c.has_dense) { if (!c.dense.bh || c.dense.cin != in_dim || c.dense.cin_pad16 > W || c.dense.N != W) return false; }
  else if (in_dim != W) return false;
  for (const ConvL& h : c.hw) if (!h.bh || !h.bh2 || h.cin != W || h.N != W) return false;
  return c.xproj.bh && c.xproj.cin == W && c.xproj.N == 6 * W;
}
static int run_chain(const taco_model* m, hipStream_t st, const Cbhg& c, const float* x, int in_dim, int M, int T, const int* lengths,
                     const CbhgWs& w, const float** ff_out, const ChainEntry* entry = nullptr) {
  ChainArgs a; memset(&a, 0, sizeof a);
  if (entry) a.e = *entry;
  a.x = x; a.ldx = in_dim; a.Cin = in_dim; a.out = w.xproj; a.ldo = 6 * c.rnn; a.rev_len = lengths; a.rev_col0 = 3 * c.rnn;
  a.M = M; a.T = T; a.krot = m->ff_rot;
  if (ff_out) { a.y = w.hi0; a.ldy = c.rnn; *ff_out = w.hi0; }
  auto add = [&](const ConvL& L, int type) {
    const GemmVar& v = m->hvars[L.var_index];
    ChainLayer& l = a.L[a.nlayers++];
    l.bh = v.bh; l.bl = v.bl; l.bh2 = v.bh2; l.bl2 = v.bl2; l.bias = v.bias; l.bias2 = v.bias2;
    l.type = type; l.K16 = v.K16; l.NT = v.NT; l.N = v.N; l.act = ACT_NONE;
  };
  if (c.has_dense) add(c.dense, CH_DENSE);
  for (int i = 0; i < c.depth; ++i) add(c.hw[i], CH_HIGHWAY);
  add(c.xproj, CH_XPROJ);
  const dim3 grid(cdiv(M, CH_BM)), blk(512);
  size_t lds = (size_t)2 * CH_BM * (c.rnn + 8) * sizeof(unsigned short);
  if (entry) lds += (size_t)2 * (CH_BM + 2) * (entry->N1 + 8) * sizeof(unsigned short);
  if (c.rnn == 256) hipLaunchKernelGGL((k_pointwise_chain<256>), grid, blk, lds, st, a);
  else hipLaunchKernelGGL((k_pointwise_chain<128>), grid, blk, lds, st, a);
  HIPCHK(hipGetLastError());
  return 0;
}

static int run_front(const taco_model* m, hipStream_t st, const Cbhg& c, const float* x, int B, int T, const CbhgWs& w, bool combine, int* P_out) {
  FrArgs a; memset(&a, 0, sizeof a);
  const int TN = c.front_kind == 1 ? 2 : 1, cinp = c.front_kind == 1 ? 80 : 128, kwmax = c.front_kind == 1 ? 8 : 16;
  const ConvL& P1 = c.proj[0];
  const GemmVar& pv = m->hvars[P1.var_index];
  a.x = x; a.ldx = c.in_dim; a.B = B; a.T = T; a.Cin = c.in_dim; a.tiles_per_b = cdiv(T, FR_BM);
  a.ph = pv.bh; a.pl = pv.bl; a.pNT = pv.NT; a.pK16tap = P1.cin_pad16 / 16;
  a.part = w.bank; a.N1 = P1.N;
  a.delay = m->front_delay;
  a.prio = m->front_prio;
  const int cpw = c.C / FR_CH, nchunks = c.K * cpw, padlmax = (kwmax - 1) / 2;
  for (int i = 0; i < c.K; ++i) {
    const ConvL& L = c.bank[i];
    FrWidth& fw = a.w[i];
    fw.wh = (const unsigned short*)AP(m, c.fr_wh[i]); fw.wl = (const unsigned short*)AP(m, c.fr_wl[i]);
    fw.bias = AP(m, L.bias); fw.scale = AP(m, L.bns); fw.shift = AP(m, L.bnb);
    fw.kw = L.kw; fw.xoff = padlmax - (L.kw - 1) / 2; fw.ns = c.fr_ns[i]; fw.nct = c.C / 16;
  }
  const int ntiles = B * a.tiles_per_b, ncu = m->cu_count > 0 ? m->cu_count : 256;
  const int pmax = std::max(1, std::min(std::min(nchunks, FR_MAXP), (c.K * c.C) / P1.N));
  int P = 1; double best = 1e30;
  for (int p = 1; p <= pmax; ++p) {
    const double cost = (double)cdiv(ntiles * p, ncu) * ((double)cdiv(nchunks, p) / nchunks + 0.03);
    if (cost < best - 1e-9) { best = cost; P = p; }
  }
  a.P = P;
  { std::vector<std::pair<long, int>> order;
    for (int i = 0; i < c.K; ++i)
      for (int j = 0; j < cpw; ++j) order.push_back({432L * c.fr_ns[i] + 4608L * TN, i * cpw + j});
    std::stable_sort(order.begin(), order.end(), [](const std::pair<long, int>& u, const std::pair<long, int>& v) { return u.first > v.first; });
    std::vector<long> load(P, 0); std::vector<std::vector<int>> mine(P);
    for (auto& o : order) {
      int tgt = 0;
      for (int p = 1; p < P; ++p) if (load[p] < load[tgt]) tgt = p;
      load[tgt] += o.first; mine[tgt].push_back(o.second);
    }
    int n = 0;
    for (int p = 0; p < P; ++p) {
      a.pstart[p] = n;
      std::sort(mine[p].begin(), mine[p].end());
      for (int id : mine[p]) {
        const int i = id / cpw, j = id % cpw;
        a.ch[n].wi = i; a.ch[n].ct0 = j * (FR_CH / 16); a.ch[n].cg0 = (c.bank[i].kw - 1) * c.C + j * FR_CH; ++n;
      }
    }
    a.pstart[P] = n; }
  const int xs = c.front_kind == 1 ? 80 : 144, xrows = c.front_kind == 1 ? 16 * FR_NRT + kwmax : FR_PR + kwmax;
  (void)cinp;
  if ((size_t)2 * xrows * xs * 2 + (size_t)2 * FR_PR * FR_ALD * 2 > FR_SMEM_CNT || (size_t)8 * 2 * TN * 16 * 64 * sizeof(float) > FR_SMEM_CNT)
    return fail(TACO_ERR_STATE, "k_cbhg_front: LDS layout does not fit");
  const size_t lds = 160 * 1024;
  const dim3 grid(ntiles * P), blk(512);
  if (c.front_kind == 1) hipLaunchKernelGGL((k_cbhg_front<2, 80, 80, 8>), grid, blk, lds, st, a);
  else hipLaunchKernelGGL((k_cbhg_front<1, 144, 128, 16>), grid, blk, lds, st, a);
  HIPCHK(hipGetLastError());
  if (P_out) *P_out = P;
  if (!combine) return 0;
  const size_t MN = (size_t)B * T * P1.N;
  hipLaunchKernelGGL(k_front_combine, dim3((unsigned)cdiv((int)(MN / 4), 256)), dim3(256), 0, st, (const float*)w.bank, P, MN, P1.N,
                     AP(m, P1.bias), AP(m, P1.bns), AP(m, P1.bnb), c.proj.size() > 1 ? 1 : 0, w.p[0]);
  HIPCHK(hipGetLastError());
  return 0;
}

struct FfProg { int w_bank = 0, w_p[4] = {0, 0, 0, 0}, w_pt = 0; };
struct FfPlan {
  GemmLevel level;
  int front_kind;
  bool entry;
  int chain_w;
  int launches;
  FfWhyNot why_front, why_entry, why_chain;
};
static FfPlan ff_plan(const taco_model* m, const Cbhg& c) {
  const ConvL& P1 = c.proj[0]; const ConvL& P2 = c.proj.back();
  FfPlan p; memset(&p, 0, sizeof p);
  p.level = gemm_level(m, P1);
  p.why_front = ff_fused_why(m, P1);
  if (!p.why_front) p.why_front = !m->front ? FF_WHY_SWITCH : c.front_kind != 0 && P1.cin == c.K * c.C && P1.cin_pad16 == c.K * c.C ? FF_WHY_NONE : FF_WHY_WIDTHS;
  p.why_chain = ff_fused_why(m, c.xproj);
  if (!p.why_chain) p.why_chain = !m->chain ? FF_WHY_SWITCH : chain_fits(c, P2.N) ? FF_WHY_NONE : FF_WHY_WIDTHS;
  p.why_entry = p.why_front || p.why_chain ? FF_WHY_NEEDS_BOTH : !m->front_entry ? FF_WHY_SWITCH :
                c.proj.size() == 2 && P2.bh && P2.kw == 3 && P2.cin == P1.N && P2.cin_pad16 == P1.N && P1.N == c.rnn && P2.N <= c.rnn && c.in_dim == P2.N
                    ? FF_WHY_NONE : FF_WHY_WIDTHS;
  p.front_kind = p.why_front ? 0 : c.front_kind; p.entry = !p.why_entry; p.chain_w = p.why_chain ? 0 : c.rnn;
  p.launches = (p.entry ? 1 : 2) + ((int)c.proj.size() - (p.entry ? 2 : 1)) + (p.chain_w ? 1 : (c.has_dense ? 1 : 0) + c.depth + 1);
  return p;
}
static int cbhg_ff_advance(const taco_model* m, hipStream_t st, const Cbhg& c, const float* x, int B, int T,
                           const int* lengths, const float* before_highway, const CbhgWs& w, FfProg& pg, int avail,
                           const float** ff_out) {
  const int M = B * T;
  auto right = [](int k) { return k - 1 - (k - 1) / 2; };
  auto advance = [&](int win, int reach) { return win >= T ? T : std::max(0, win - reach); };
  const FfPlan fp = ff_plan(m, c);
  const bool front = fp.front_kind && avail >= T && pg.w_bank == 0 && pg.w_p[0] == 0, entry = front && fp.entry;
  int parts = 1;
  if (front) {
    TRY(run_front(m, st, c, x, B, T, w, !entry, &parts));
    pg.w_bank = T; pg.w_p[0] = T;
    if (entry) pg.w_p[1] = T;
  }
  { const int nw = advance(avail, right(c.K));
    if (nw > pg.w_bank) {
      GemmCall g; g.x = x; g.ldx = c.in_dim; g.M = M; g.T = T; g.act = ACT_RELU; g.out = w.bank; g.ldo = c.K * c.C;
      g.t_begin = pg.w_bank; g.t_len = nw - pg.w_bank;
      TRY(run_gemm(m, st, c.bank.data(), c.K, false, g));
      pg.w_bank = nw;
    } }
  const float* cur = w.bank; int curd = c.K * c.C;
  for (size_t i = 0; i < c.proj.size(); ++i) {
    const int win = (i == 0) ? pg.w_bank : pg.w_p[i - 1];
    const int nw = advance(win, right(c.pw) + ((i == 0) ? right(c.maxpool) : 0));
    if (nw > pg.w_p[i]) {
      GemmCall p;
      p.x = cur; p.ldx = curd; p.M = M; p.T = T; p.mpw = (i == 0) ? c.maxpool : 1;
      p.act = (i + 1 == c.proj.size()) ? ACT_NONE : ACT_RELU;
      p.out = w.p[i]; p.ldo = c.proj[i].N;
      p.t_begin = pg.w_p[i]; p.t_len = nw - pg.w_p[i];
      if (i + 1 == c.proj.size()) {
        p.res = x; p.ldres = c.in_dim;
        p.rowvec = before_highway; p.ldrv = c.in_dim;
      }
      TRY(run_gemm(m, st, &c.proj[i], 1, false, p));
      pg.w_p[i] = nw;
    }
    cur = w.p[i]; curd = c.proj[i].N;
  }
  const int wlast = pg.w_p[c.proj.size() - 1];
  const int t0 = pg.w_pt, tl = wlast - pg.w_pt;
  if (fp.chain_w && t0 == 0 && tl == T) {
    ChainEntry E; memset(&E, 0, sizeof E);
    if (entry) {
      const ConvL& P1 = c.proj[0]; const ConvL& P2 = c.proj[1];
      const GemmVar& v2 = m->hvars[P2.var_index];
      E.part = w.bank; E.P = parts; E.MN = (size_t)M * P1.N; E.N1 = P1.N;
      E.b1 = AP(m, P1.bias); E.s1 = AP(m, P1.bns); E.h1 = AP(m, P1.bnb); E.relu1 = 1;
      E.bh = v2.bh; E.bl = v2.bl; E.NT2 = v2.NT; E.K16tap = P2.cin_pad16 / 16; E.N2 = P2.N;
      E.b2 = AP(m, P2.bias); E.s2 = AP(m, P2.bns); E.h2 = AP(m, P2.bnb);
      E.res = x; E.ldres = c.in_dim; E.rowvec = before_highway; E.ldrv = c.in_dim;
    }
    TRY(run_chain(m, st, c, cur, curd, M, T, lengths, w, ff_out, entry ? &E : nullptr));
    pg.w_pt = wlast;
    return 0;
  }
  if (c.has_dense) {
    if (tl > 0) { GemmCall d; d.x = cur; d.ldx = curd; d.M = M; d.T = T; d.out = w.hi0; d.ldo = c.rnn; d.t_begin = t0; d.t_len = tl;
      TRY(run_gemm(m, st, &c.dense, 1, false, d)); }
    cur = w.hi0;
  }
  float* bufs[2] = {w.hi0, w.hi1};
  int sel = (cur == w.hi0) ? 1 : 0;
  for (int i = 0; i < c.depth; ++i) {
    if (tl > 0) { GemmCall h; h.x = cur; h.ldx = c.rnn; h.M = M; h.T = T; h.out = bufs[sel]; h.ldo = c.rnn; h.t_begin = t0; h.t_len = tl;
      TRY(run_gemm(m, st, &c.hw[i], 1, true, h)); }
    cur = bufs[sel]; sel ^= 1;
  }
  if (tl > 0) {
    const int H = c.rnn;
    GemmCall xp; xp.x = cur; xp.ldx = c.rnn; xp.M = M; xp.T = T; xp.out = w.xproj; xp.ldo = 6 * H;
    xp.rev_len = lengths; xp.rev_col0 = 3 * H; xp.t_begin = t0; xp.t_len = tl;
    TRY(run_gemm(m, st, &c.xproj, 1, false, xp));
    pg.w_pt = wlast;
  }
  if (ff_out) *ff_out = cur;
  return 0;
}

static int cbhg_forward(const taco_model* m, hipStream_t st, const Cbhg& c, const float* x, int B, int T,
                        const int* lengths, const float* before_highway, const float* init_state, float* out,
                        const CbhgWs& w) {
  FfProg pg;
  TRY(cbhg_ff_advance(m, st, c, x, B, T, lengths, before_highway, w, pg, T, nullptr));
  return bigru_scan(m, st, c, B, T, lengths, init_state, out, w);
}

struct SpkWs { float *emb, *vec[8]; };
static void carve_spk(Carver& cv, const taco_model* m, int B, SpkWs& w) {
  const taco_hparams& hp = m->hp;
  w.emb = cv.f((size_t)B * std::max(hp.speaker_embedding_size, 1));
  const int dims[3] = {hp.enc_prenet[hp.enc_prenet_n - 1], hp.enc_rnn_size * 2, hp.attention_state_size};
  for (int i = 0; i < 3 + hp.dec_layer_num; ++i) w.vec[i] = cv.f((size_t)B * (i < 3 ? dims[i] : hp.dec_rnn_size));
}
static bool is_deepvoice(const taco_model* m) { return m->hp.num_speakers > 1 && m->hp.model_type == 2; }
static bool is_simple(const taco_model* m) { return m->hp.num_speakers > 1 && m->hp.model_type == 1; }
static int simple_S(const taco_model* m) { return is_simple(m) ? m->hp.speaker_embedding_size : 0; }
static int spk_forward(const taco_model* m, hipStream_t st, const int* speaker_id, int B, const SpkWs& w) {
  const taco_hparams& hp = m->hp;
  const int nv = 3 + hp.dec_layer_num;
  const int dims[3] = {hp.enc_prenet[hp.enc_prenet_n - 1], hp.enc_rnn_size * 2, hp.attention_state_size};
  if (hp.speaker_embedding_size == 1) {
    for (int i = 0; i < nv; ++i) {
      const int D = i < 3 ? dims[i] : hp.dec_rnn_size;
      hipLaunchKernelGGL(k_gather_rows, dim3(cdiv(B * D, 256)), dim3(256), 0, st, AP(m, m->spk_table[i]), speaker_id, B, D, w.vec[i]);
    }
    HIPCHK(hipGetLastError());
    return 0;
  }
  const int S = hp.speaker_embedding_size;
  hipLaunchKernelGGL(k_gather_rows, dim3(cdiv(B * S, 256)), dim3(256), 0, st, AP(m, m->spk_emb), speaker_id, B, S, w.emb);
  HIPCHK(hipGetLastError());
  for (int i0 = 0; i0 < nv; i0 += SK_MAXJOBS) {
    SkJob js[SK_MAXJOBS];
    const int nj = std::min(SK_MAXJOBS, nv - i0);
    for (int i = 0; i < nj; ++i) {
      const int D = (i0 + i) < 3 ? dims[i0 + i] : hp.dec_rnn_size;
      js[i] = sk_linear(m, m->spk_dense[i0 + i], w.emb, S, S, nullptr, 0, ACT_SOFTSIGN, w.vec[i0 + i], D);
    }
    TRY(run_skinny(st, B, js, nj));
  }
  return 0;
}

struct EncWs { float* pre[4]; CbhgWs cb; SpkWs spk; };
static void carve_enc(Carver& cv, const taco_model* m, int B, int T, EncWs& w) {
  for (int i = 0; i < m->hp.enc_prenet_n; ++i) w.pre[i] = cv.f((size_t)B * T * m->hp.enc_prenet[i]);
  carve_cbhg(cv, m->enc, B, T, w.cb);
  carve_spk(cv, m, B, w.spk);
}
static FfWhyNot prenet_chain_why(const taco_model* m) {
  const taco_hparams& hp = m->hp;
  if (const FfWhyNot why = ff_fused_why(m, m->enc_prenet[0])) return why;
  if (!m->chain) return FF_WHY_SWITCH;
  if (hp.enc_prenet_n != 2) return FF_WHY_WIDTHS;
  const ConvL& a = m->enc_prenet[0]; const ConvL& b = m->enc_prenet[1];
  return b.bh && a.kw == 1 && b.kw == 1 && a.N == 256 && a.cin == hp.embedding_size && a.cin_pad16 <= 256 && (hp.embedding_size & 3) == 0 &&
         b.cin == 256 && b.N == hp.enc_prenet[1] && a.var_index >= 0 && b.var_index >= 0 ? FF_WHY_NONE : FF_WHY_WIDTHS;
}
static int run_prenet_chain(const taco_model* m, hipStream_t st, const int* ids, int M, float* out, const ZeroRegions* riders) {
  const taco_hparams& hp = m->hp;
  ChainArgs a; memset(&a, 0, sizeof a);
  a.x = AP(m, m->emb); a.ldx = hp.embedding_size; a.Cin = hp.embedding_size; a.gather = ids;
  a.out = out; a.ldo = hp.enc_prenet[1]; a.rev_len = nullptr; a.rev_col0 = -1; a.M = M; a.T = M; a.krot = m->ff_rot;
  const int types[2] = {CH_DENSE, CH_XPROJ};
  for (int i = 0; i < 2; ++i) {
    const GemmVar& v = m->hvars[m->enc_prenet[i].var_index];
    ChainLayer& l = a.L[a.nlayers++];
    l.bh = v.bh; l.bl = v.bl; l.bh2 = v.bh2; l.bl2 = v.bl2; l.bias = v.bias; l.bias2 = v.bias2;
    l.type = types[i]; l.K16 = v.K16; l.NT = v.NT; l.N = v.N; l.act = ACT_RELU;
  }
  int nwg = cdiv(M, CH_BM);
  if (riders) {
    a.ntiles = nwg;
    for (int i = 0; i < 4; ++i) { a.zp[i] = riders->p[i]; a.znw[i] = riders->nw[i]; }
    nwg += std::min(192, std::max(16, 256 - nwg));
  }
  hipLaunchKernelGGL((k_pointwise_chain<256>), dim3(nwg), dim3(512), (size_t)2 * CH_BM * (256 + 8) * sizeof(unsigned short), st, a);
  HIPCHK(hipGetLastError());
  if (riders) register_cleared(*riders);
  return 0;
}
static int encoder_forward(const taco_model* m, hipStream_t st, const int* ids, const int* lengths, const int* speaker_id,
                           int B, int T, float* enc_out, const EncWs& w, bool spk_done, bool prenet_chain, const ZeroRegions* riders = nullptr) {
  const taco_hparams& hp = m->hp;
  const int M = B * T;
  if (is_deepvoice(m) && !spk_done) TRY(spk_forward(m, st, speaker_id, B, w.spk));
  const float* cur = AP(m, m->emb); int curd = hp.embedding_size;
  if (prenet_chain) {
    TRY(run_prenet_chain(m, st, ids, M, w.pre[1], riders));
    return cbhg_forward(m, st, m->enc, w.pre[1], B, T, lengths, is_deepvoice(m) ? w.spk.vec[0] : nullptr,
                        is_deepvoice(m) ? w.spk.vec[1] : nullptr, enc_out, w.cb);
  }
  for (int i = 0; i < hp.enc_prenet_n; ++i) {
    GemmCall g; g.x = cur; g.ldx = curd; g.gather = (i == 0) ? ids : nullptr; g.M = M; g.act = ACT_RELU;
    g.out = w.pre[i]; g.ldo = hp.enc_prenet[i];
    TRY(run_gemm(m, st, &m->enc_prenet[i], 1, false, g));
    cur = w.pre[i]; curd = hp.enc_prenet[i];
  }
  return cbhg_forward(m, st, m->enc, cur, B, T, lengths, is_deepvoice(m) ? w.spk.vec[0] : nullptr,
                      is_deepvoice(m) ? w.spk.vec[1] : nullptr, enc_out, w.cb);
}

struct DecWs {
  float *keys, *zero, *ctx, *pz[4], *h_att, *rh, *u, *xc, *q, *align, *o[5], *hd[4], *Y, *escr;
  int* nz;
  unsigned long long* xbuf; size_t xbuf_bytes; unsigned* dxctl;
  float* rowbias;
  SpkWs spk;
};
static void carve_dec(Carver& cv, const taco_model* m, int B, int T_in, int n, DecWs& w) {
  const taco_hparams& hp = m->hp;
  const int D = 2 * hp.enc_rnn_size, As = hp.attention_state_size, Hd = hp.dec_rnn_size;
  const int Hmax = std::max(As, Hd);
  w.keys = cv.f((size_t)B * T_in * hp.attention_size);
  w.zero = cv.f((size_t)B * hp.num_mels);
  const int S = simple_S(m);
  w.h_att = cv.f((size_t)B * (As + D + S)); w.ctx = w.h_att ? w.h_att + As : nullptr;
  for (int i = 0; i < hp.dec_prenet_n; ++i) w.pz[i] = cv.f((size_t)B * (hp.dec_prenet[i] + S));
  w.rh = cv.f((size_t)B * Hmax); w.u = cv.f((size_t)B * Hmax); w.xc = cv.f((size_t)B * 2 * Hmax);
  w.q = cv.f((size_t)B * hp.attention_size);
  w.align = cv.f((size_t)B * T_in);
  w.escr = cv.f((size_t)B * T_in);
  for (int i = 0; i <= hp.dec_layer_num; ++i) w.o[i] = cv.f((size_t)B * Hd);
  for (int i = 0; i < hp.dec_layer_num; ++i) w.hd[i] = cv.f((size_t)B * Hd);
  w.Y = nullptr;
  w.nz = cv.i((size_t)n * B);
  carve_spk(cv, m, B, w.spk);
  {
    w.xbuf_bytes = (size_t)DX_NGROUP * dx_xlayout(8, T_in).total * sizeof(unsigned long long);
    w.xbuf = (unsigned long long*)cv.raw(w.xbuf_bytes);
    w.dxctl = (unsigned*)cv.raw(256);
    w.rowbias = cv.f(is_simple(m) ? (size_t)B * DXRB_N * DX_W : 1);
  }
}
static constexpr size_t DX_LDS_BUDGET = 160 * 1024;
enum DecUse { DEC_INFER, DEC_TEACHER, DEC_TRAIN_FWD, DEC_TRAIN_BWD };
enum DecWhyNot { DEC_WHY_NONE, DEC_WHY_ENGINE_OFF, DEC_WHY_CUS, DEC_WHY_ROWS, DEC_WHY_WIDTHS, DEC_WHY_TEACHER_ROWS, DEC_WHY_NO_INSTANTIATION, DEC_WHY_LDS, DEC_WHY_TAPE_LAYOUT };
static_assert((int)DEC_WHY_ENGINE_OFF == SCAN_WHY_ENGINE_OFF && (int)DEC_WHY_CUS == SCAN_WHY_CUS && (int)DEC_WHY_ROWS == SCAN_WHY_ROWS, "taco_model_engine_plan words the shared reasons once");
struct DecPlan {
  bool persistent;
  int rg, aw, pd;
  bool tape;
  size_t lds_bytes;
  DecWhyNot why;
};
static DecPlan decoder_plan(const taco_model* m, int B, int T_in, int n, DecUse use) {
  const taco_hparams& hp = m->hp;
  const bool bwd = use == DEC_TRAIN_BWD, train = bwd || use == DEC_TRAIN_FWD;
  DecPlan p = {false, 0, hp.attention_size, dx_prenet_depth(m), use != DEC_INFER, 0, DEC_WHY_NONE};
  const int lo = dx_reference_widths(m) ? 1 : 4;
  for (p.rg = lo; p.rg < 8 && p.rg * DX_NGROUP < B; p.rg *= 2) {}
  if (m->dx_rows >= lo && m->dx_rows * DX_NGROUP >= B) p.rg = m->dx_rows;
  p.lds_bytes = (bwd ? db_lds_floats(p.rg, T_in) : dx_lds_floats(p.rg, T_in, p.tape, p.aw)) * sizeof(float);
  if (!m->dx_mode) p.why = DEC_WHY_ENGINE_OFF;
  else if (m->cu_count < CHIP_CUS) p.why = DEC_WHY_CUS;
  else if (B > CHIP_ROWS) p.why = DEC_WHY_ROWS;
  else if (!(bwd ? m->dbx_pack : m->dx_pack)) p.why = DEC_WHY_WIDTHS;
  else if (use == DEC_TEACHER && !m->tp && !(m->dx_p1o_raw && hp.num_mels <= DX_P2)) p.why = DEC_WHY_TEACHER_ROWS;
  else if (p.aw == 512 && p.rg > 4) p.why = DEC_WHY_NO_INSTANTIATION;
  else if (p.lds_bytes > DX_LDS_BUDGET) p.why = DEC_WHY_LDS;
  else if (train && ((!bwd && hp.num_mels > DX_P2) || (size_t)DXT_N * B * n * DX_W >= (1u << 31))) p.why = DEC_WHY_TAPE_LAYOUT;
  p.persistent = p.why == DEC_WHY_NONE;
  return p;
}
template <int RG, bool TAPE, int AW = DX_W, int PD = 2>
static int dx_launch_rg(hipStream_t st, const DxArgs& a_in, size_t lds) {
  DxArgs a = a_in;
  if constexpr (!TAPE && AW == DX_W && PD == 2) {
    if (a.trace && !a.manual) { hipLaunchKernelGGL((k_decoder_xcd<RG, false, false, AW, PD, true>), dim3(CHIP_CUS), dim3(DX_NT), lds, st, a); HIPCHK(hipGetLastError()); return 0; }
  }
  a.trace = nullptr;
  if (a.manual) { hipLaunchKernelGGL((k_decoder_xcd<RG, TAPE, true, AW, PD>), dim3(CHIP_CUS), dim3(DX_NT), lds, st, a); HIPCHK(hipGetLastError()); return 0; }
  hipLaunchKernelGGL((k_decoder_xcd<RG, TAPE, false, AW, PD>), dim3(CHIP_CUS), dim3(DX_NT), lds, st, a);
  HIPCHK(hipGetLastError());
  return 0;
}
#define DX_REFERENCE(X) X(1, false, DX_W, 2) X(2, false, DX_W, 2) X(4, false, DX_W, 2) X(8, false, DX_W, 2)
#define DX_REFERENCE_TAPE(X) X(1, true, DX_W, 2) X(2, true, DX_W, 2) X(4, true, DX_W, 2) X(8, true, DX_W, 2)
#define DX_PRESETS(X) X(4, false, 128, 2) X(8, false, 128, 2) X(4, false, 256, 3) X(8, false, 256, 3) X(4, false, 512, 3) X(4, false, 128, 3) X(8, false, 128, 3) X(4, false, 512, 2)
static constexpr int dx_inst(int rg, bool tape, int aw, int pd) { return rg | (tape ? 16 : 0) | pd << 8 | aw << 12; }
static int dx_launch(const taco_model* m, hipStream_t st, const DecPlan& dp, const float* enc_out, const int* speaker_id, const float* spk_rows, int B, int T_in, int n,
                     const float* manual, float* mel, float* align_out, float* dbg, int dbgw, const float* keys, int* nz,
                     unsigned long long* xbuf, unsigned* dxctl, float* rowbias, const float* h_att0, const float* h10, const float* h20,
                     const DxArgs* tape = nullptr) {
  ChipTurn turn(m->device, st);
#ifdef DX_DLY_RT
  {
    int d[32]; const int dflt[11] = {DX_POLL_DELAY_B, DX_FIRST_POLL_DELAY, DX_FIRST_POLL_DELAY, DX_FIRST_POLL_DELAY, DX_POLL_DELAY_B, DX_FIRST_POLL_DELAY,
                                     DX_FIRST_POLL_DELAY, DX_POLL_DELAY_B, DX_FIRST_POLL_DELAY, DX_POLL_DELAY_B, DX_FIRST_POLL_DELAY};
    for (int i = 0; i < 32; ++i) d[i] = (i & 15) < 11 ? dx_site_delay(i & 15, dflt[i & 15], dp.rg) : 0;
    if (const char* e = getenv("TACO_DX_DLY")) { int i = 0; const char* p = e; while (*p && i < 11) { d[i] = d[16 + i] = atoi(p); ++i; while (*p && *p != ',') ++p; if (*p == ',') ++p; } }
    if (const char* e = getenv("TACO_DX_DLY_B")) { int i = 0; const char* p = e; while (*p && i < 11) { d[16 + i] = atoi(p); ++i; while (*p && *p != ',') ++p; if (*p == ',') ++p; } }
    HIPCHK(hipMemcpyToSymbol(HIP_SYMBOL(g_dx_dly), d, sizeof d));
  }
#endif
  DxArgs a; memset(&a, 0, sizeof a);
  if (tape) a = *tape;
  a.manual = manual;
  if (is_simple(m)) {
    hipLaunchKernelGGL(k_dx_rowbias, dim3(B), dim3(DX_W), 0, st, spk_rows ? spk_rows : AP(m, m->spk_emb), spk_rows ? (const int*)nullptr : speaker_id,
                       AP(m, m->dx_spkw), m->hp.speaker_embedding_size, rowbias);
    HIPCHK(hipGetLastError());
    a.rowbias = rowbias;
  }
  a.wpack = AP(m, m->dx_pack);
  a.qpack = AP(m, m->dx_qpack[dp.rg == 1 ? 0 : dp.rg == 2 ? 1 : dp.rg == 4 ? 2 : 3]);
  a.b_p1_0 = AP(m, m->dx_b_p1_0); a.b_p1c = AP(m, m->dx_b_p1c); a.b_p2 = AP(m, m->dx_b_p2); a.b_p3 = AP(m, m->dx_b_p3); a.b_ag = AP(m, m->dx_b_ag); a.b_ac = AP(m, m->dx_b_ac);
  a.b_g1f = AP(m, m->dx_b_g1f); a.b_g1c = AP(m, m->dx_b_g1c); a.b_g2g = AP(m, m->dx_b_g2g); a.b_g2c = AP(m, m->dx_b_g2c);
  a.b_f = AP(m, m->dx_b_f);
  a.att_v = AP(m, m->att_v); a.att_b = AP(m, m->att_b); a.score_bias = AP(m, m->att_sb);
  a.keys = keys; a.values = enc_out; a.h_att0 = h_att0; a.h10 = h10; a.h20 = h20;
  a.mel = mel; a.hist = align_out; a.nz = nz; a.dbg = dbg; a.dbgw = dbgw;
  a.xbuf = xbuf; a.ctl = dxctl; a.err = m->d_err; a.trace = m->trace_on ? m->d_trace : nullptr;
  if (a.trace) { const char* e = getenv("TACO_TRACE_MEMBER"); a.trc_member = e ? atoi(e) : 0; e = getenv("TACO_TRACE_TID"); a.trc_tid = e ? atoi(e) : 0; }
  a.B = B; a.T_in = T_in; a.n = n; a.rM = m->hp.num_mels * m->hp.reduction_factor; a.att_type = m->hp.attention_type;
  a.mels = m->hp.num_mels;
  a.grp0 = 0; a.ngroups = cdiv(B, dp.rg); a.force_wt = m->dx_mode == 2 ? 1 : 0;
  HIPCHK(clear_polled(xbuf, (size_t)((char*)dxctl - (char*)xbuf) + 256, st));
  switch (dx_inst(dp.rg, dp.tape, dp.aw, dp.pd)) {
#define X(RG, TAPE, AW, PD) case dx_inst(RG, TAPE, AW, PD): return dx_launch_rg<RG, TAPE, AW, PD>(st, a, dp.lds_bytes);
    DX_REFERENCE(X) DX_REFERENCE_TAPE(X) DX_PRESETS(X)
#undef X
    default: return fail(TACO_ERR_STATE, "no persistent decoder instantiation for attention_size %d, %d prenet layers, %d rows per group%s", dp.aw, dp.pd, dp.rg, dp.tape ? ", tape" : "");
  }
}
static size_t dbx_xbuf_granules(int T_in) {
  size_t g = 0;
  for (int RG = 1; RG <= 8; RG *= 2) g = std::max(g, (size_t)db_xlayout(RG, T_in).total);
  return g;
}
// ... 410 lines not shown
    m->skinny[n] = m->dec_prenet.back();
    d = hp.dec_prenet[i];
  }
  m->att_gru = make_grudec(m, "decoder/attention_gru", d + simple_S(m), As);
  m->grus["decoder/attention_gru"] = m->att_gru;
  m->query = pack_w16(m, T_(m, "attention/query_layer/kernel").data.data(), A, 0, As, 0, A, nullptr);
  m->skinny["attention/query_layer"] = m->query;
  m->raw_wq = arena_put(m, T_(m, "attention/query_layer/kernel").data.data(), (size_t)As * A);
  m->concat_proj = pack_w16(m, T_(m, "decoder/concat_projection/kernel").data.data(), Hd, 0, As + D + simple_S(m), 0, Hd, T_(m, "decoder/concat_projection/bias").data.data());
  m->skinny["decoder/concat_projection"] = m->concat_proj;
  for (int i = 0; i < hp.dec_layer_num; ++i) {
    const std::string n = "decoder/gru_" + std::to_string(i + 1);
    m->dec_gru.push_back(make_grudec(m, n, Hd, Hd));
    m->grus[n] = m->dec_gru.back();
  }
  const int rM = hp.num_mels * hp.reduction_factor;
  m->frame_proj = pack_w16(m, T_(m, "decoder/frame_projection/kernel").data.data(), rM, 0, Hd, 0, rM, T_(m, "decoder/frame_projection/bias").data.data());
  m->skinny["decoder/frame_projection"] = m->frame_proj;
  std::vector<float> dx_Wc, dx_bc;
  {
    const int Mm = hp.num_mels, P0 = hp.dec_prenet[0];
    const auto& Wf = T_(m, "decoder/frame_projection/kernel").data; const auto& bf = T_(m, "decoder/frame_projection/bias").data;
    const auto& W1 = T_(m, "decoder/prenet/dense_1/kernel").data; const auto& b1 = T_(m, "decoder/prenet/dense_1/bias").data;
    std::vector<float>& Wc = dx_Wc; std::vector<float>& bc = dx_bc;
    Wc.assign((size_t)(Hd + D) * P0, 0.f); bc.assign(P0, 0.f);
    for (int k = 0; k < Hd; ++k)
      for (int q = 0; q < P0; ++q) {
        double acc = 0;
        for (int j = 0; j < Mm; ++j) acc += (double)Wf[(size_t)k * rM + (rM - Mm) + j] * (double)W1[(size_t)j * P0 + q];
        Wc[(size_t)k * P0 + q] = (float)acc;
      }
    for (int k = 0; k < D; ++k)
      for (int q = 0; q < P0; ++q) Wc[(size_t)(Hd + k) * P0 + q] = W1[(size_t)(Mm + k) * P0 + q];
    for (int q = 0; q < P0; ++q) {
      double acc = b1[q];
      for (int j = 0; j < Mm; ++j) acc += (double)bf[(rM - Mm) + j] * (double)W1[(size_t)j * P0 + q];
      bc[q] = (float)acc;
    }
    m->prenet1_next = pack_w16(m, Wc.data(), P0, 0, Hd + D, 0, P0, bc.data());
  }
  if (!m->tp && hp.dec_layer_num > 0) {
    const int Z = As + D + simple_S(m), N4 = 4 * Hd;
    const auto& Wc = T_(m, "decoder/concat_projection/kernel").data; const auto& bcv = T_(m, "decoder/concat_projection/bias").data;
    const auto& gk = T_(m, "decoder/gru_1/gates/kernel").data; const auto& gb = T_(m, "decoder/gru_1/gates/bias").data;
    const auto& ck = T_(m, "decoder/gru_1/candidate/kernel").data; const auto& cb = T_(m, "decoder/gru_1/candidate/bias").data;
    std::vector<float> W((size_t)(Z + Hd) * N4, 0.f), bb(N4, 0.f);
    std::vector<double> row(3 * Hd);
    for (int z = 0; z <= Z; ++z) {
      std::fill(row.begin(), row.end(), 0.0);
      for (int k = 0; k < Hd; ++k) {
        const double c = (z < Z) ? (double)Wc[(size_t)z * Hd + k] : (double)bcv[k];
        for (int j = 0; j < 2 * Hd; ++j) row[j] += c * (double)gk[(size_t)k * 2 * Hd + j];
        for (int j = 0; j < Hd; ++j) row[2 * Hd + j] += c * (double)ck[(size_t)k * Hd + j];
      }
      if (z < Z) {
        for (int j = 0; j < 3 * Hd; ++j) W[(size_t)z * N4 + j] = (float)row[j];
        for (int j = 0; j < Hd; ++j) W[(size_t)z * N4 + 3 * Hd + j] = Wc[(size_t)z * Hd + j];
      } else {
        for (int j = 0; j < 2 * Hd; ++j) bb[j] = (float)(row[j] + (double)gb[j]);
        for (int j = 0; j < Hd; ++j) { bb[2 * Hd + j] = (float)row[2 * Hd + j]; bb[3 * Hd + j] = bcv[j]; }
      }
    }
    for (int k = 0; k < Hd; ++k)
      for (int j = 0; j < 2 * Hd; ++j) W[(size_t)(Z + k) * N4 + j] = gk[(size_t)(Hd + k) * 2 * Hd + j];
    m->gru1_fold.I = Z; m->gru1_fold.H = Hd;
    m->gru1_fold.gx = pack_w16(m, W.data(), N4, 0, Z + Hd, 0, N4, bb.data());
    m->gru1_fold.ch = pack_w16(m, ck.data(), Hd, Hd, Hd, 0, Hd, cb.data());
    m->fuse_concat = 1;
    if (hp.dec_layer_num == 2) TRY(dx_build_pack(m, dx_Wc, dx_bc, W, bb));
  }
  if (m->tp && hp.dec_layer_num == 2 && dx_widths_ok(m)) {
    const int Mm = hp.num_mels, P0 = hp.dec_prenet[0], H = Hd, Z = As + D + simple_S(m), N4 = 4 * H;
    const auto& W1 = T_(m, "decoder/prenet/dense_1/kernel").data;
    std::vector<float> Wc_t((size_t)(Hd + D) * P0, 0.f);
    for (int k = 0; k < Mm; ++k) for (int q = 0; q < P0; ++q) Wc_t[(size_t)k * P0 + q] = W1[(size_t)k * P0 + q];
    for (int k = 0; k < D; ++k) for (int q = 0; q < P0; ++q) Wc_t[(size_t)(Hd + k) * P0 + q] = W1[(size_t)(Mm + k) * P0 + q];
    const auto& Wcc = T_(m, "decoder/concat_projection/kernel").data; const auto& bcv = T_(m, "decoder/concat_projection/bias").data;
    const auto& gk = T_(m, "decoder/gru_1/gates/kernel").data;
    size_t NP = 0;
    for (auto& sp : m->spec) { size_t c = 1; for (int64_t d : sp.second) c *= (size_t)d; NP += c; }
    std::vector<float> Wf_t((size_t)(Z + Hd) * N4, 0.f), bf_t(N4, 0.f);
    for (int z = 0; z <= Z; ++z)
      for (int j = 0; j < 3 * H; ++j) {
        const float idx = (float)(NP + 1 + (size_t)z * 3 * H + j);
        if (z < Z) Wf_t[(size_t)z * N4 + j] = idx; else bf_t[j] = idx;
      }
    for (int z = 0; z < Z; ++z) for (int j = 0; j < H; ++j) Wf_t[(size_t)z * N4 + 3 * H + j] = Wcc[(size_t)z * Hd + j];
    for (int j = 0; j < H; ++j) bf_t[3 * H + j] = bcv[j];
    for (int k = 0; k < Hd; ++k) for (int j = 0; j < 2 * H; ++j) Wf_t[(size_t)(Z + k) * N4 + j] = gk[(size_t)(Hd + k) * 2 * H + j];
    m->dx_fold_n = (size_t)(Z + 1) * 3 * H;
    if (NP + m->dx_fold_n >= (1u << 24)) return fail(TACO_ERR_UNSUPPORTED, "parameter + fold indices exceed 2^24");
    TRY(dx_build_pack(m, Wc_t, T_(m, "decoder/prenet/dense_1/bias").data, Wf_t, bf_t));
    TRY(dbx_build_pack(m));
  }
  {
    std::vector<float> v = T_(m, "attention/attention_v").data;
    if (hp.attention_type == 1) {
      double nrm = 0; for (float x : v) nrm += (double)x * x;
      const double sc = (double)T_(m, "attention/attention_g").data[0] / std::sqrt(nrm);
      for (float& x : v) x = (float)(x * sc);
      m->att_b = arena_put(m, T_(m, "attention/attention_b").data.data(), A);
    }
    m->att_v = arena_put(m, v.data(), A);
    if (hp.attention_type == 2) m->att_sb = arena_put(m, T_(m, "attention/attention_score_bias").data.data(), 1);
  }
  if (is_deepvoice(m)) {
    std::vector<std::string> names = {kSpkNames[0], kSpkNames[1], kSpkNames[2]};
    for (int i = 0; i < hp.dec_layer_num; ++i) names.push_back("decoder_rnn_init_" + std::to_string(i + 1));
    if (hp.speaker_embedding_size == 1) {
      for (auto& n : names) m->spk_table.push_back(arena_put(m, T_(m, "spk/" + n + "/table").data.data(), T_(m, "spk/" + n + "/table").data.size()));
    } else {
      m->spk_emb = arena_put(m, T_(m, "speaker_embedding").data.data(), T_(m, "speaker_embedding").data.size());
      for (auto& n : names) {
        const HostTensor& k = T_(m, "spk/" + n + "/kernel");
        m->spk_dense.push_back(pack_w16(m, k.data.data(), (int)k.shape[1], 0, (int)k.shape[0], 0, (int)k.shape[1], T_(m, "spk/" + n + "/bias").data.data()));
      }
    }
  }
  for (int i = 0; i < hp.enc_prenet_n; ++i) add_var(m, m->enc_prenet[i], 0);
  for (Cbhg* c : {&m->enc, &m->post}) {
    for (size_t i = 0; i < c->bank.size(); ++i) add_var(m, c->bank[i], (c->bank[i].kw - 1) * c->C);
    for (auto& L : c->proj) add_var(m, L, 0);
    if (c->has_dense) add_var(m, c->dense, 0);
    for (auto& L : c->hw) add_var(m, L, 0);
    add_var(m, c->xproj, 0);
  }
  add_var(m, m->memory_layer, 0);
  add_var(m, m->linear, 0);
  for (auto& kv : m->convs) add_var(m, kv.second, 0);
  for (int i = 0; i < hp.enc_prenet_n; ++i) m->convs["prenet/dense_" + std::to_string(i + 1)] = m->enc_prenet[i];
  m->convs["attention/memory_layer"] = m->memory_layer;
  m->convs["linear"] = m->linear;
  if (m->tp) TRY(build_train_packs(m));
  HIPCHK(hipMalloc((void**)&m->darena, m->harena.size() * sizeof(float)));
  HIPCHK(hipMemcpy(m->darena, m->harena.data(), m->harena.size() * sizeof(float), hipMemcpyHostToDevice));
  for (auto& v : m->hvars) {
    v.wp = AP(m, (size_t)v.wp); v.wp2 = AP(m, (size_t)v.wp2); v.bias = AP(m, (size_t)v.bias); v.bias2 = AP(m, (size_t)v.bias2);
    v.bn_scale = AP(m, (size_t)v.bn_scale); v.bn_shift = AP(m, (size_t)v.bn_shift);
    v.bh = (const unsigned short*)AP(m, (size_t)v.bh); v.bl = (const unsigned short*)AP(m, (size_t)v.bl);
    v.bh2 = (const unsigned short*)AP(m, (size_t)v.bh2); v.bl2 = (const unsigned short*)AP(m, (size_t)v.bl2);
    v.bl3 = (const unsigned short*)AP(m, (size_t)v.bl3); v.bl3_2 = (const unsigned short*)AP(m, (size_t)v.bl3_2);
  }
  HIPCHK(hipFuncSetAttribute(reinterpret_cast<const void*>(&k_cbhg_front<2, 80, 80, 8>), hipFuncAttributeMaxDynamicSharedMemorySize, 160 * 1024));
  HIPCHK(hipFuncSetAttribute(reinterpret_cast<const void*>(&k_cbhg_front<1, 144, 128, 16>), hipFuncAttributeMaxDynamicSharedMemorySize, 160 * 1024));
  HIPCHK(hipFuncSetAttribute(reinterpret_cast<const void*>(&k_bigru_res<256, 64, 24, 1, false>), hipFuncAttributeMaxDynamicSharedMemorySize, 160 * 1024));
  HIPCHK(hipFuncSetAttribute(reinterpret_cast<const void*>(&k_bigru_res<128, 32, 0, 1, false>), hipFuncAttributeMaxDynamicSharedMemorySize, 160 * 1024));
  HIPCHK(hipFuncSetAttribute(reinterpret_cast<const void*>(&k_bigru_res<256, 64, 24, 1, true>), hipFuncAttributeMaxDynamicSharedMemorySize, 160 * 1024));
  HIPCHK(hipFuncSetAttribute(reinterpret_cast<const void*>(&k_bigru_res<128, 32, 0, 1, true>), hipFuncAttributeMaxDynamicSharedMemorySize, 160 * 1024));
  HIPCHK(hipFuncSetAttribute(reinterpret_cast<const void*>(&k_bigru_resw<16, 4, 2>), hipFuncAttributeMaxDynamicSharedMemorySize, 160 * 1024));
  HIPCHK(hipFuncSetAttribute(reinterpret_cast<const void*>(&k_bigru_rows<1, false>), hipFuncAttributeMaxDynamicSharedMemorySize, 160 * 1024));
  HIPCHK(hipFuncSetAttribute(reinterpret_cast<const void*>(&k_bigru_rows<2, false>), hipFuncAttributeMaxDynamicSharedMemorySize, 160 * 1024));
  HIPCHK(hipFuncSetAttribute(reinterpret_cast<const void*>(&k_bigru_rows<1, true>), hipFuncAttributeMaxDynamicSharedMemorySize, 160 * 1024));
  HIPCHK(hipFuncSetAttribute(reinterpret_cast<const void*>(&k_bigru_rows<2, true>), hipFuncAttributeMaxDynamicSharedMemorySize, 160 * 1024));
  HIPCHK(hipFuncSetAttribute(reinterpret_cast<const void*>(&k_pointwise_chain<256>), hipFuncAttributeMaxDynamicSharedMemorySize, 160 * 1024));
  HIPCHK(hipFuncSetAttribute(reinterpret_cast<const void*>(&k_head_sweep<512>), hipFuncAttributeMaxDynamicSharedMemorySize, 160 * 1024));
  HIPCHK(hipFuncSetAttribute(reinterpret_cast<const void*>(&k_head_sweep<256>), hipFuncAttributeMaxDynamicSharedMemorySize, 160 * 1024));
  HIPCHK(hipFuncSetAttribute(reinterpret_cast<const void*>(&k_pointwise_chain<128>), hipFuncAttributeMaxDynamicSharedMemorySize, 160 * 1024));
  TRY(gemm_set_attributes());
#define DX_ATTR(...) HIPCHK(hipFuncSetAttribute(reinterpret_cast<const void*>(&k_decoder_xcd<__VA_ARGS__>), hipFuncAttributeMaxDynamicSharedMemorySize, DX_LDS_BUDGET));
#define PLAIN(RG, TAPE, AW, PD) DX_ATTR(RG, TAPE, false, AW, PD)
#define MANUAL(RG, TAPE, AW, PD) DX_ATTR(RG, TAPE, true, AW, PD)
#define BOTH(RG, TAPE, AW, PD) PLAIN(RG, TAPE, AW, PD) MANUAL(RG, TAPE, AW, PD)
#define STAMPED(RG, TAPE, AW, PD) DX_ATTR(RG, TAPE, false, AW, PD, true)
  DX_REFERENCE(PLAIN) DX_REFERENCE(MANUAL) DX_REFERENCE_TAPE(BOTH) DX_REFERENCE(STAMPED) DX_PRESETS(BOTH)
#undef DX_ATTR
#undef PLAIN
#undef MANUAL
#undef BOTH
#undef STAMPED
  HIPCHK(hipStreamCreateWithFlags(&m->side, hipStreamNonBlocking));
  m->events.resize(192);
  for (auto& e : m->events) HIPCHK(hipEventCreateWithFlags(&e, hipEventDisableTiming));
  HIPCHK(hipMalloc((void**)&m->d_err, 256));
  HIPCHK(hipMemset(m->d_err, 0, 256));
  m->arena_n = m->harena.size();
  m->harena.clear(); m->harena.shrink_to_fit();
  m->raw.clear();
  m->finalized = true;
  return 0;
}

void taco_model_destroy(taco_model* m) {
  if (!m) return;
  if (m->darena) (void)hipFree(m->darena);
  if (m->d_err) (void)hipFree(m->d_err);
  if (m->d_trace) (void)hipFree(m->d_trace);
  for (auto& e : m->events) (void)hipEventDestroy(e);
  if (m->side) (void)hipStreamDestroy(m->side);
  delete m;
}

int taco_model_device_errors(taco_model* m, int* out) {
  if (!m || !m->finalized || !out) return fail(TACO_ERR_ARG, "bad argument");
  HIPCHK(hipSetDevice(m->device));
  unsigned v = 0;
  HIPCHK(hipMemcpy(&v, m->d_err, sizeof v, hipMemcpyDeviceToHost));
  if (v) HIPCHK(hipMemset(m->d_err, 0, 256));
  *out = (int)v;
  return 0;
}

int taco_debug_raise_device_error(taco_model* m, int value) {
  if (!m || !m->finalized) return fail(TACO_ERR_ARG, "bad argument");
  HIPCHK(hipSetDevice(m->device));
  const unsigned v = (unsigned)value;
  HIPCHK(hipMemcpy(m->d_err, &v, sizeof v, hipMemcpyHostToDevice));
  return 0;
}

int taco_debug_set_bf3(taco_model* m, int on, int tile_n) {
  if (!m) return fail(TACO_ERR_ARG, "null model");
  if (!gemm_tile_known(tile_n)) return fail(TACO_ERR_ARG, "tile_n is not one of 0, 4, 5, 7, 9, 10");
  m->bf3 = (on & 1) != 0; m->bf3_tn = tile_n;
  m->chain = (on & 4) ? 0 : 1;
  m->front = (on & 8) ? 0 : 1;
  m->front_entry = (on & 16) ? 0 : 1;
  m->head_sweep = (on & 32) ? 0 : 1;
  if (!m->tp) m->bf3x6 = (on & 64) ? 1 : 0;
  return 0;
}

int taco_attention_trim(void* hip_stream, const float* d_alignments, const int32_t* d_seq_len, int B, int T_in, int n_steps,
                        int reduction_factor, int32_t* d_spec_end) {
  if (!d_alignments || !d_seq_len || !d_spec_end || B <= 0 || T_in <= 0 || n_steps <= 0) return fail(TACO_ERR_ARG, "bad argument");
  if ((size_t)n_steps * sizeof(int) > 64 * 1024) return fail(TACO_ERR_UNSUPPORTED, "more than 16384 decoder steps");
  hipLaunchKernelGGL(k_attention_trim, dim3(B), dim3(64), (size_t)n_steps * sizeof(int), (hipStream_t)hip_stream, d_alignments, d_seq_len, T_in,
                     n_steps, reduction_factor, d_spec_end);
  HIPCHK(hipGetLastError());
  return 0;
}

int taco_stop_steps(void* hip_stream, const float* d_mel, int B, int n_steps, int width, int rows_per_group, int32_t* d_stop) {
  if (!d_mel || !d_stop || B <= 0 || n_steps <= 0 || width <= 0 || rows_per_group <= 0 || B % rows_per_group)
    return fail(TACO_ERR_ARG, "bad argument");
  hipStream_t st = (hipStream_t)hip_stream;
  HIPCHK(zero_async(d_stop, (size_t)(B / rows_per_group) * sizeof(int32_t), st));
  hipLaunchKernelGGL(k_stop_groups, dim3(B), dim3(256), 0, st, d_mel, n_steps, width, rows_per_group, d_stop);
  HIPCHK(hipGetLastError());
  return 0;
}

int taco_model_set_batch_invariant(taco_model* m, int on) {
  if (!m) return fail(TACO_ERR_ARG, "null model");
  m->ff_rot = on ? 0 : 1;
  return 0;
}
int taco_debug_set_att_split(taco_model* m, int slices) {
  if (!m) return fail(TACO_ERR_ARG, "null model");
  m->att_split = slices;
  return 0;
}
int taco_debug_set_fuse_prenet(taco_model* m, int on) {
  if (!m) return fail(TACO_ERR_ARG, "null model");
  m->fuse_prenet1 = on ? 1 : 0;
  return 0;
}
#ifdef TACO_TRACE
int taco_debug_read_trace(long long* out) { return hipMemcpyFromSymbol(out, HIP_SYMBOL(taco_trace), 64 * sizeof(long long)) == hipSuccess ? 0 : -1; }
int taco_debug_read_trace_front(long long* out) { return hipMemcpyFromSymbol(out, HIP_SYMBOL(taco_trace_front), 64 * sizeof(long long)) == hipSuccess ? 0 : -1; }
int taco_debug_read_trace_head(long long* out) { return hipMemcpyFromSymbol(out, HIP_SYMBOL(taco_trace_head), 16 * sizeof(long long)) == hipSuccess ? 0 : -1; }
int taco_debug_read_trace_chain(long long* out) { return hipMemcpyFromSymbol(out, HIP_SYMBOL(taco_trace_chain), 64 * sizeof(long long)) == hipSuccess ? 0 : -1; }
#endif
int taco_debug_set_fuse_concat(taco_model* m, int on) {
  if (!m) return fail(TACO_ERR_ARG, "null model");
  if (on && !m->gru1_fold.H) return fail(TACO_ERR_STATE, "the folded GRU pack was not built for this model");
  m->fuse_concat = on ? 1 : 0;
  return 0;
}
int taco_debug_set_overlap(taco_model* m, int on) {
  if (!m) return fail(TACO_ERR_ARG, "null model");
  m->overlap = on;
  return 0;
}

int taco_debug_set_persistent(taco_model* m, int on) {
  if (!m) return fail(TACO_ERR_ARG, "null model");
  switch (on) {
    case SCAN_PER_STEP: case SCAN_AUTO: case SCAN_ROWS: case SCAN_RES: case SCAN_RESW: case SCAN_OCT: case SCAN_DUO: break;
    default: return fail(TACO_ERR_ARG, "scan mode %d: accepted are 0 (two launches per step), 1 (default: the fastest kernel that fits), 2 (k_bigru_rows), "
                                       "3 (k_bigru_res), 7 (k_bigru_resw), 10 (k_bigru_oct wherever it fits), 11 (k_bigru_duo, never k_bigru_oct)", on);
  }
  m->persist = on;
  return 0;
}

int taco_debug_set_decoder_persist(taco_model* m, int mode, int rows_per_group) {
  if (!m) return fail(TACO_ERR_ARG, "null model");
  if (mode < 0 || mode > 2) return fail(TACO_ERR_ARG, "mode must be 0 (launch per stage), 1 (persistent) or 2 (persistent, write-through exchanges)");
  if (rows_per_group != 0 && rows_per_group != 1 && rows_per_group != 2 && rows_per_group != 4 && rows_per_group != 8)
    return fail(TACO_ERR_ARG, "rows_per_group %d: accepted are 0 (the smallest that covers the batch), 1, 2, 4 and 8", rows_per_group);
  m->dx_mode = mode; m->dx_rows = rows_per_group;
  return 0;
}
int taco_debug_decoder_info(taco_model* m, int* out16) {
  if (!m || !m->finalized || !out16) return fail(TACO_ERR_ARG, "bad argument");
  HIPCHK(hipSetDevice(m->device));
  unsigned v[16];
  HIPCHK(hipMemcpy(v, m->d_err + 8, sizeof v, hipMemcpyDeviceToHost));
  for (int i = 0; i < 16; ++i) out16[i] = (int)v[i];
  { unsigned b = 0; HIPCHK(hipMemcpy(&b, m->d_err + 40, sizeof b, hipMemcpyDeviceToHost)); out16[9] = m->last_bptt ? (int)b : 0; }
  out16[14] = m->cu_count;
  out16[15] = m->dx_pack ? 1 : 0;
  return 0;
}
int taco_model_engine_plan(taco_model* m, int B, int T_in, int T_mel, int flags, char* out, int out_len) {
  if (!m || !m->finalized || !out || out_len < 64) return fail(TACO_ERR_ARG, "bad argument");
  std::string s;
  const int cap = decoder_pass_rows(m, (flags & 4) != 0), n = std::max(1, T_mel / std::max(1, m->hp.reduction_factor));
  if (B > cap && !m->tp) {
    const PassPlan pp = pass_plan(B, cap);
    s = std::to_string(B) + " rows = " + std::to_string(pp.passes) + " passes of " + std::to_string(pp.rows) + " (the last one " + std::to_string(B - (pp.passes - 1) * pp.rows) + "); per pass: ";
    B = pp.rows;
  }
  auto why_common = [&](int why, int rows) -> std::string {
    if (why == DEC_WHY_ENGINE_OFF) return "switched off (taco_debug_set_decoder_persist 0)";
    if (why == DEC_WHY_CUS) return "the device exposes " + std::to_string(m->cu_count) + " compute units (a partition of an MI355X, or another part): the whole-chip kernels need 256";
    return why == DEC_WHY_ROWS ? std::to_string(rows) + " rows > 64 per launch" : "";
  };
  auto dec_why = [&](const DecPlan& dp) -> std::string {
    switch (dp.why) {
      case DEC_WHY_WIDTHS: return "widths outside the presets (256-wide decoder cells and memory, attention_size 128 / 256 / 512, prenet 256-128[-64], 2 decoder layers, r * num_mels <= 512)";
      case DEC_WHY_TEACHER_ROWS: return "teacher frames on an inference model outside the reference widths (attention_size 256, prenet 256-128, num_mels <= 128)";
      case DEC_WHY_NO_INSTANTIATION: return "attention_size 512 with more than 32 rows (no instantiation at 8 rows per group)";
      case DEC_WHY_LDS: return "T_in = " + std::to_string(T_in) + " does not fit a member's LDS at " + std::to_string(dp.rg) + " rows per group";
      case DEC_WHY_TAPE_LAYOUT: return "a tape of " + std::to_string(B) + " rows x " + std::to_string(n) + " steps at num_mels " + std::to_string(m->hp.num_mels) + " is outside the kernel's layout (num_mels <= 128, 20 x rows x steps x 256 < 2^31)";
      default: return why_common(dp.why, B);
    }
  };
  {
    const DecPlan dp = decoder_plan(m, B, T_in, n, m->tp ? DEC_TRAIN_FWD : (flags & 2) ? DEC_TEACHER : DEC_INFER);
    const int chunk = m->tp || (flags & 6) ? 0 : overlap_chunk(m, n);
    if (dp.persistent && !chunk)
      s += "decoder loop: persistent k_decoder_xcd<" + std::to_string(dp.rg) + (dx_reference_widths(m) ? std::string("") : ", attention " + std::to_string(dp.aw) + ", " +
           std::to_string(dp.pd) + " prenet layers") + "> (" + std::string((flags & 1) ? "manual alignments" : "computed alignments") + ", " +
           std::string(m->dx_mode == 2 ? "write-through exchanges forced" : "XCD-local exchanges when the census finds 32 workgroups per XCD") + ")";
    else s += "decoder loop: one launch per stage -- " + (dp.persistent ? "taco_debug_set_overlap: the post-net's feed-forward stages follow the loop in chunks of " + std::to_string(chunk) + " steps" : dec_why(dp));
  }
  auto scan_why = [&](const Cbhg& c, const ScanPlan& sp, const char* width_name, int rows) -> std::string {
    switch (sp.why_not_whole_chip) {
      case SCAN_WHY_MODE: return "taco_debug_set_persistent(" + std::to_string(m->persist) + "): " + scan_kernel_name(sp.kernel);
      case SCAN_WHY_WIDTH: return std::string(width_name) + " " + std::to_string(c.rnn) + " != 256";
      case SCAN_WHY_FRAMES: return "fewer than 2 frames";
      default: return why_common(sp.why_not_whole_chip, rows);
    }
  };
  {
    const Cbhg& c = m->post;
    const ScanPlan sp = scan_plan(m, c, B, T_mel, m->tp != nullptr);
    if (sp.kernel == SCAN_K_OCT) s += "; post-net scan: persistent k_bigru_oct<" + std::to_string(sp.upw) + "> (one row per cluster of " + std::to_string(DX_GROUP / sp.upw) + " CUs)";
    else if (sp.kernel == SCAN_K_DUO) s += "; post-net scan: persistent k_bigru_duo<" + std::to_string(sp.rg) + ">";
    else if (sp.kernel == SCAN_K_QUAD) s += "; post-net scan: k_bigru_quad (post_rnn_size 128: a row and direction per workgroup, its weights resident, no exchange between workgroups)";
    else s += "; post-net scan: resident per-row kernels -- " + scan_why(c, sp, "post_rnn_size", B);
  }
  {
    const Cbhg& c = m->enc;
    const ScanPlan sp = scan_plan(m, c, B, T_in, m->tp != nullptr);
    if (sp.kernel == SCAN_K_OCT) s += "; encoder scan: persistent k_bigru_oct<" + std::to_string(sp.upw) + ">";
    else if (sp.kernel == SCAN_K_DUO) s += "; encoder scan: persistent k_bigru_duo<" + std::to_string(sp.rg) + ">";
    else if (sp.kernel == SCAN_K_QUAD) s += "; encoder scan: k_bigru_quad (a row and direction per workgroup, K split inside a quad of lanes)";
    else if (sp.kernel == SCAN_K_RES || sp.kernel == SCAN_K_RESW) s += std::string("; encoder scan: ") + scan_kernel_name(sp.kernel) + " (rows resident per workgroup)";
    else s += std::string("; encoder scan: ") + scan_kernel_name(sp.kernel);
    s += "; feed-forward: ";
  }
  const int chunk = m->tp || (flags & 6) ? 0 : overlap_chunk(m, n);
  auto gemm_name = [](GemmLevel lv) { return lv == GEMM_BF3 ? "k_gemm_bf3" : lv == GEMM_BF3X6 ? "k_gemm_bf3<..., X6>" : "k_gemm"; };
  auto launches = [](int k) { return std::to_string(k) + (k == 1 ? " launch" : " launches"); };
  auto ff_why = [&](const char* kernel, FfWhyNot why, int bit, const char* widths = "widths outside the presets") -> std::string {
    static const char* const words[] = {"", "exact fp32 is switched on", "the six-product level has no fused kernels", "taco_debug_force_gemm_config", "a k_gemm_bf3 tile is forced"};
    return std::string(" -- no ") + kernel + ": " + (why == FF_WHY_SWITCH ? "taco_debug_set_bf3 bit " + std::to_string(bit) : why == FF_WHY_WIDTHS ? std::string(widths) : std::string(words[why]));
  };
  auto cbhg_ff = [&](const char* name, const Cbhg& c, bool chunked) -> std::string {
    const FfPlan fp = ff_plan(m, c);
    const int per_layer = 1 + (int)c.proj.size() + (c.has_dense ? 1 : 0) + c.depth + 1;
    std::string r = std::string("; ") + name + " CBHG: ";
    if (m->tp) return r + launches(per_layer) + " of " + gemm_name(fp.level) + ", one per layer";
    if (chunked) return r + launches(per_layer) + " of " + gemm_name(fp.level) + " per chunk, one per layer (taco_debug_set_overlap)";
    r += launches(fp.launches) + ": ";
    r += fp.front_kind == 1 ? "k_cbhg_front<2, 80, 80, 8>" : fp.front_kind ? "k_cbhg_front<1, 144, 128, 16>" : std::string("conv bank and proj_1 on ") + gemm_name(fp.level);
    if (fp.front_kind && !fp.entry) r += " + k_front_combine";
    if (const int np = (int)c.proj.size() - (fp.entry ? 2 : 1)) r += ", " + std::to_string(np) + (np == 1 ? " projection on " : " projections on ") + gemm_name(fp.level);
    if (fp.chain_w) r += ", k_pointwise_chain<" + std::to_string(fp.chain_w) + ">" + (fp.entry ? " (the last projection in its entry)" : "");
    else r += ", " + std::to_string(fp.launches - 1 - (int)c.proj.size()) + " point-wise layers on " + gemm_name(fp.level);
    if (fp.why_front) r += ff_why("k_cbhg_front", fp.why_front, 3);
    if (fp.why_chain) r += ff_why("k_pointwise_chain", fp.why_chain, 2);
    if (fp.why_entry && fp.why_entry != FF_WHY_NEEDS_BOTH) r += ff_why("fused chain entry", fp.why_entry, 4);
    return r;
  };
  { const GemmLevel lv = gemm_level(m, m->linear);
    s += lv == GEMM_BF3 ? "split-bf16 MFMA, three products (k_gemm_bf3 and the fused kernels)" : lv == GEMM_BF3X6 ? "split-bf16 MFMA, six products (k_gemm_bf3<..., X6>: fp32-grade)" : "exact-fp32 MFMA (k_gemm)";
    s += cbhg_ff("encoder", m->enc, false) + cbhg_ff("post-net", m->post, chunk != 0);
    const FfWhyNot pw = prenet_chain_why(m);
    if (!m->tp && !pw) s += std::string("; encoder prenet: one k_pointwise_chain launch (1 launch: embedding rows gathered, both layers") + (chunk ? ")" : "; the forward's zero fills ride in it)");
    else s += "; encoder prenet: one GEMM launch per layer (" + launches(m->hp.enc_prenet_n) + " of " + gemm_name(gemm_level(m, m->enc_prenet[0])) +
              (m->tp ? ")" : std::string(chunk ? "" : " + 1 launch of k_zero_fill_multi in front: the forward's zero fills") + ff_why("k_pointwise_chain", pw, 2) + ")");
    GemmCall g; g.ldx = 2 * m->hp.post_rnn_size; g.M = B * T_mel; g.ldo = m->hp.num_freq;
    const FfWhyNot hw = head_sweep_why(m, m->linear, 1, false, g);
    s += std::string("; linear head: 1 launch of ") + (hw ? gemm_name(lv) + ff_why("k_head_sweep", hw, 5, "it serves 256 rows and more, 256 or 512 inputs, 512 columns and more") :
                                                                m->linear.cin == 512 ? "k_head_sweep<512>" : "k_head_sweep<256>"); }
  if (m->tp) {
    const Cbhg& c = m->post;
    const ScanBwd bwd = scan_plan(m, c, B, T_mel).bwd;
    s += std::string("; backward scans: post-net ") + (bwd == SCAN_BWD_OCT ? "k_bigru_oct_bwd (one row per cluster of 8 CUs)" : bwd == SCAN_BWD_DUO ? "k_bigru_duo_bwd" : "k_bigru_rows_bwd") +
         ", encoder " + (m->enc.rnn == 128 ? "k_bigru_resb (recurrent kernels in registers)" : "k_bigru_rows_bwd");
    const DecPlan bp = decoder_plan(m, B, T_in, n, DEC_TRAIN_BWD);
    s += "; decoder backward loop: " + (bp.persistent ? "persistent k_decoder_bwd_xcd<" + std::to_string(bp.rg) + ">" : "one launch per stage -- " + dec_why(bp));
  }
  snprintf(out, (size_t)out_len, "%s", s.c_str());
  return 0;
}
int taco_debug_decoder_trace(taco_model* m, int enable, long long* out) {
  if (!m || !m->finalized) return fail(TACO_ERR_ARG, "bad argument");
  HIPCHK(hipSetDevice(m->device));
  const size_t half = (size_t)DX_TRACE_STEPS * DX_TRACE_SLOTS * sizeof(long long);
  if ((enable & 1) && !m->d_trace) { HIPCHK(hipMalloc((void**)&m->d_trace, 3 * half)); HIPCHK(hipMemset(m->d_trace, 0, 3 * half)); }
  if (out && m->d_trace) HIPCHK(hipMemcpy(out, (const char*)m->d_trace + ((enable & 4) ? 2 * half : (enable & 2) ? half : 0), half, hipMemcpyDeviceToHost));
  m->trace_on = enable & 1;
  return 0;
}

int taco_debug_set_front(taco_model* m, int delay_clocks, int prio) {
  if (!m) return fail(TACO_ERR_ARG, "null model");
  m->front_delay = delay_clocks; m->front_prio = prio;
  return 0;
}
int taco_debug_set_chip_turns(int on) { g_chip_turns = on ? 1 : 0; return 0; }
int taco_debug_set_skip_scans(taco_model* m, int on) {
  if (!m) return fail(TACO_ERR_ARG, "null model");
  m->skip_scans = on ? 1 : 0;
  return 0;
}

int taco_debug_force_gemm_config(taco_model* m, int cfg) {
  if (!m) return fail(TACO_ERR_ARG, "null model");
  if (!gemm_cfg_known(cfg)) return fail(TACO_ERR_ARG, "cfg is not one of -1, 1, 2");
  m->force_cfg = cfg;
  return 0;
}

size_t taco_workspace_bytes(const taco_model* m, int B, int T_in, int n_steps) {
  if (!m || B <= 0) return 0;
  return forward_workspace(m, B, T_in, n_steps, nullptr, nullptr, nullptr, 0, nullptr);
}

size_t taco_stage_workspace_bytes(const taco_model* m, int B, int T) {
  if (!m) return 0;
  Carver a(nullptr, 0), b(nullptr, 0), c(nullptr, 0);
  const int R = B > 64 ? pass_plan(B).rows : B;
  const int cap = decoder_pass_rows(m), Rd = B > cap ? pass_plan(B, cap).rows : B;
  EncWs e; carve_enc(a, m, R, T, e);
  DecWs d; carve_dec(b, m, Rd, T, T, d);
  PostWs p; carve_post(c, m, R, T, p);
  return std::max(a.off, std::max(b.off, c.off)) + (B > cap ? 256 : 0);
}

int taco_forward_infer(taco_model* m, void* hip_stream, const int32_t* d_inputs, const int32_t* d_input_lengths,
                       const int32_t* d_speaker_id, int B, int T_in, int n_steps, const float* d_manual_alignments,
                       float* d_mel, float* d_linear, float* d_alignments, int32_t* d_stop_step, void* d_workspace,
                       size_t workspace_bytes) {
  if (m) HIPCHK(hipSetDevice(m->device));
  return forward_enqueue(m, (hipStream_t)hip_stream, d_inputs, d_input_lengths, d_speaker_id, B, T_in, n_steps,
                         d_manual_alignments, d_mel, d_linear, d_alignments, d_stop_step, d_workspace, workspace_bytes);
}

struct taco_plan {
  hipGraph_t graph = nullptr;
  hipGraphExec_t exec = nullptr;
  size_t nodes = 0;
  int device = 0;
  bool whole_chip = false;
};

int taco_plan_create(taco_model* m, const int32_t* d_inputs, const int32_t* d_input_lengths, const int32_t* d_speaker_id,
                     int B, int T_in, int n_steps, const float* d_manual_alignments, float* d_mel, float* d_linear,
                     float* d_alignments, int32_t* d_stop_step, void* d_workspace, size_t workspace_bytes, taco_plan** out) {
  if (!m || !out) return fail(TACO_ERR_ARG, "null argument");
  HIPCHK(hipSetDevice(m->device));
  hipStream_t cs;
  HIPCHK(hipStreamCreateWithFlags(&cs, hipStreamNonBlocking));
  hipError_t e = hipStreamBeginCapture(cs, hipStreamCaptureModeThreadLocal);
  if (e != hipSuccess) { (void)hipStreamDestroy(cs); return fail(TACO_ERR_HIP, "hipStreamBeginCapture: %s", hipGetErrorString(e)); }
  g_captured_whole_chip = false;
  int rc = forward_enqueue(m, cs, d_inputs, d_input_lengths, d_speaker_id, B, T_in, n_steps, d_manual_alignments, d_mel,
                           d_linear, d_alignments, d_stop_step, d_workspace, workspace_bytes);
  const bool whole_chip = g_captured_whole_chip;
  hipGraph_t g = nullptr;
  e = hipStreamEndCapture(cs, &g);
  (void)hipStreamDestroy(cs);
  if (rc != 0) { if (g) (void)hipGraphDestroy(g); return rc; }
  if (e != hipSuccess) return fail(TACO_ERR_HIP, "hipStreamEndCapture: %s", hipGetErrorString(e));
  taco_plan* p = new taco_plan();
  p->graph = g; p->device = m->device; p->whole_chip = whole_chip;
  e = hipGraphInstantiate(&p->exec, g, nullptr, nullptr, 0);
  if (e != hipSuccess) { (void)hipGraphDestroy(g); delete p; return fail(TACO_ERR_HIP, "hipGraphInstantiate: %s", hipGetErrorString(e)); }
  (void)hipGraphGetNodes(g, nullptr, &p->nodes);
  *out = p;
  return 0;
}

int taco_plan_launch(taco_plan* p, void* hip_stream) {
  if (!p || !p->exec) return fail(TACO_ERR_ARG, "null plan");
  if (p->whole_chip) {
    ChipTurn turn(p->device, (hipStream_t)hip_stream);
    HIPCHK(hipGraphLaunch(p->exec, (hipStream_t)hip_stream));
    return 0;
  }
  HIPCHK(hipGraphLaunch(p->exec, (hipStream_t)hip_stream));
  return 0;
}
int taco_plan_num_nodes(const taco_plan* p) { return p ? (int)p->nodes : 0; }
int taco_plan_whole_chip(const taco_plan* p) { return (p && p->whole_chip) ? 1 : 0; }
void taco_plan_destroy(taco_plan* p) {
  if (!p) return;
  if (p->exec) (void)hipGraphExecDestroy(p->exec);
  if (p->graph) (void)hipGraphDestroy(p->graph);
  delete p;
}

int taco_encoder_forward(taco_model* m, void* hip_stream, const int32_t* d_inputs, const int32_t* d_input_lengths,
                         const int32_t* d_speaker_id, int B, int T_in, float* d_encoder_out, void* d_workspace,
                         size_t workspace_bytes) {
  if (m && m->finalized && B > 64 && T_in > 0 && d_inputs && d_input_lengths && d_encoder_out) {
    const PassPlan pp = pass_plan(B);
    for (int b0 = 0; b0 < B; b0 += pp.rows)
      TRY(taco_encoder_forward(m, hip_stream, d_inputs + (size_t)b0 * T_in, d_input_lengths + b0, d_speaker_id ? d_speaker_id + b0 : nullptr, std::min(pp.rows, B - b0),
                               T_in, d_encoder_out + (size_t)b0 * T_in * 2 * m->hp.enc_rnn_size, d_workspace, workspace_bytes));
    return 0;
  }
  TRY(check_common(m, B, T_in));
  if (!d_inputs || !d_input_lengths || !d_encoder_out || !d_workspace) return fail(TACO_ERR_ARG, "null buffer");
  if (m->hp.num_speakers > 1 && !d_speaker_id) return fail(TACO_ERR_ARG, "speaker_id required for a multi-speaker model");
  HIPCHK(hipSetDevice(m->device));
  Carver cv(d_workspace, workspace_bytes);
  EncWs w; carve_enc(cv, m, B, T_in, w);
  if (!cv.ok()) return fail(TACO_ERR_STATE, "workspace too small: need %zu bytes", cv.off);
  return encoder_forward(m, (hipStream_t)hip_stream, d_inputs, d_input_lengths, d_speaker_id, B, T_in, d_encoder_out, w, false, prenet_chain_why(m) == FF_WHY_NONE);
}

int taco_decoder_forward(taco_model* m, void* hip_stream, const float* d_encoder_out, const int32_t* d_speaker_id, int B,
                         int T_in, int n_steps, const float* d_manual_alignments, const float* d_teacher_frames,
                         float* d_mel, float* d_alignments, int32_t* d_stop_step, float* d_dbg_states, void* d_workspace,
                         size_t workspace_bytes) {
  if (m && m->finalized && B > decoder_pass_rows(m, d_dbg_states != nullptr) && T_in > 0 && n_steps > 0 && d_encoder_out && d_mel && d_alignments && d_workspace) {
    if (d_dbg_states) return fail(TACO_ERR_UNSUPPORTED, "the per-step state dump is laid out [step][row]: at most 64 rows per call");
    const PassPlan pp = pass_plan(B, decoder_pass_rows(m));
    const size_t rM = (size_t)m->hp.reduction_factor * m->hp.num_mels, D = (size_t)2 * m->hp.enc_rnn_size;
// ... 203 lines not shown
```

Before: 6.407 million.

## Add 32-row tiles to pointwise chain kernel for small batches with wave-role split

Templates k_pointwise_chain on tile rows and adds a 32-row variant, chosen automatically when the row count yields at most 128 tiles, so small problems launch more workgroups to fill the GPU. In the 32-row, width-128 case the waves split into two roles. For highway layers one role computes the gate GEMM and hands it to the other through an LDS exchange buffer, and xproj column groups are divided between the roles. The trade is smaller tiles with more weight reloads per row and an extra barrier and LDS exchange. The highway epilogue is also reworked with explicit FMA control to keep its numerics.

```diff
diff --git a/include/taco_debug.h b/include/taco_debug.h
--- a/include/taco_debug.h
+++ b/include/taco_debug.h
@@ -14,6 +14,7 @@
 int taco_debug_set_fuse_prenet(taco_model* m, int on);
 int taco_debug_set_fuse_concat(taco_model* m, int on);
 int taco_debug_set_att_split(taco_model* m, int slices);
+int taco_debug_set_chain_rows(taco_model* m, int rows);
 int taco_debug_set_overlap(taco_model* m, int on);
 
 int taco_debug_set_decoder_persist(taco_model* m, int mode, int rows_per_group);
diff --git a/multi-speaker-tacotron-tensorflow_amd/_lib.py b/multi-speaker-tacotron-tensorflow_amd/_lib.py
--- a/multi-speaker-tacotron-tensorflow_amd/_lib.py
+++ b/multi-speaker-tacotron-tensorflow_amd/_lib.py
@@ -189,6 +189,7 @@
     "taco_debug_set_fuse_prenet": (_I, [_P, _I]),
     "taco_debug_set_fuse_concat": (_I, [_P, _I]),
     "taco_debug_set_att_split": (_I, [_P, _I]),
+    "taco_debug_set_chain_rows": (_I, [_P, _I]),
     "taco_debug_set_bf3": (_I, [_P, _I, _I]),
     "taco_model_device_errors": (_I, [_P, C.POINTER(_I)]),
     "taco_debug_raise_device_error": (_I, [_P, _I]),
diff --git a/multi-speaker-tacotron-tensorflow_amd/csrc/taco_chain.h b/multi-speaker-tacotron-tensorflow_amd/csrc/taco_chain.h
--- a/multi-speaker-tacotron-tensorflow_amd/csrc/taco_chain.h
+++ b/multi-speaker-tacotron-tensorflow_amd/csrc/taco_chain.h
@@ -11,7 +11,11 @@
 #ifndef CH_ROT
 #define CH_ROT 1
 #endif
-#define CH_BM 64
+constexpr int ch_roles(int W, int BM) { return (256 / W) > (BM / 32) ? (256 / W) / (BM / 32) : 1; }
+constexpr size_t ch_xchg_shorts(int W, int BM) { return ch_roles(W, BM) == 2 ? (size_t)(W / 32) * 16 * 64 * 2 : 0; }
+constexpr size_t ch_lds_bytes(int W, int BM, int N1) {
+  return ((size_t)2 * BM * (W + 8) + ch_xchg_shorts(W, BM) + (N1 ? (size_t)2 * (BM + 2) * (N1 + 8) : 0)) * sizeof(unsigned short);
+}
 enum { CH_DENSE = 0, CH_HIGHWAY = 1, CH_XPROJ = 2 };
 struct ChainLayer {
   const unsigned short* bh; const unsigned short* bl; const unsigned short* bh2; const unsigned short* bl2;
@@ -114,21 +118,23 @@
 #else
 #define CTRC(i) do {} while (0)
 #endif
-template <int W>
+template <int W, int BM>
 __global__ __launch_bounds__(512) void k_pointwise_chain(const ChainArgs a_in) {
-  constexpr int WN = W / 32, WM = 8 / WN, TM = CH_BM / 32 / WM;
+  static_assert((W == 256 || W == 128) && (BM == 64 || BM == 32), "k_pointwise_chain: no such instantiation");
+  constexpr int WN = W / 32, ROLES = ch_roles(W, BM), WM = 8 / WN / ROLES, TM = BM / 32 / WM;
   constexpr int PF = W == 256 ? CH_PF256 : CH_PF128;
   constexpr int LDSW = W + 8;
   extern __shared__ __attribute__((aligned(16))) unsigned short ch_smem[];
   unsigned short* xhi = ch_smem;
-  unsigned short* xlo = ch_smem + CH_BM * LDSW;
+  unsigned short* xlo = ch_smem + BM * LDSW;
   struct { const float* x; float* out; float* y; const int* rev_len; int ldx, Cin, ldo, ldy, rev_col0, M, T, nlayers; } a =
       {a_in.x, a_in.out, a_in.y, a_in.rev_len, a_in.ldx, a_in.Cin, a_in.ldo, a_in.ldy, a_in.rev_col0, a_in.M, a_in.T, a_in.nlayers};
   PIN(a.x); PIN(a.out); PIN(a.y); PIN(a.rev_len); PIN(a.ldx); PIN(a.Cin); PIN(a.ldo); PIN(a.ldy); PIN(a.rev_col0); PIN(a.M); PIN(a.T);
   PIN(a.nlayers);
   const int tid = threadIdx.x, lane = tid & 63, l31 = lane & 31, lh = lane >> 5;
   const int wave = __builtin_amdgcn_readfirstlane(tid >> 6);
-  const int wm = wave / WN, wn = wave % WN;
+  const int wn = wave % WN, wm = ROLES == 2 ? 0 : wave / WN, role = ROLES == 2 ? wave / WN : 0;
+  const bool own = role == 0;
   if (a_in.ntiles > 0 && (int)blockIdx.x >= a_in.ntiles) {
     const size_t i0 = (size_t)((int)blockIdx.x - a_in.ntiles) * 512 + tid, stride = (size_t)((int)gridDim.x - a_in.ntiles) * 512;
     for (int rg = 0; rg < 4; ++rg) {
@@ -142,7 +148,7 @@
     }
     return;
   }
-  const int m0 = blockIdx.x * CH_BM;
+  const int m0 = blockIdx.x * BM;
   const int krot = (CH_ROT && a_in.krot) ? ((int)(blockIdx.x >> 3) & 31) : 0;
 #ifdef TACO_TRACE
   const bool trc = (blockIdx.x == (a_in.ntiles > 0 ? a_in.ntiles : gridDim.x) / 2) && threadIdx.x == 0;
@@ -160,10 +166,10 @@
     const float* gres = E.res; const float* grv = E.rowvec; const float* gb2 = E.b2; const float* gs2 = E.s2; const float* gh2 = E.h2;
     PIN(gpart); PIN(gb1); PIN(gs1); PIN(gh1); PIN(gbh); PIN(gbl); PIN(gres); PIN(grv); PIN(gb2); PIN(gs2); PIN(gh2);
     const int LDE = E.N1 + 8;
-    unsigned short* ehi = ch_smem + 2 * CH_BM * LDSW;
-    unsigned short* elo = ehi + (CH_BM + 2) * LDE;
+    unsigned short* ehi = ch_smem + 2 * BM * LDSW + ch_xchg_shorts(W, BM);
+    unsigned short* elo = ehi + (BM + 2) * LDE;
     const int nq = E.N1 / 4;
-    constexpr int NSTG = ((CH_BM + 2) * (256 / 4) + 511) / 512;
+    constexpr int NSTG = ((BM + 2) * (256 / 4) + 511) / 512;
     {
       float4 f[NSTG];
       const float* src[NSTG];
@@ -171,7 +177,7 @@
       for (int u = 0; u < NSTG; ++u) {
         const int i = tid + 512 * u, r = i / nq, c = 4 * (i - r * nq), row = m0 - 1 + r;
         f[u] = make_float4(0.f, 0.f, 0.f, 0.f);
-        src[u] = (i < (CH_BM + 2) * nq && row >= 0 && row < a.M) ? gpart + (size_t)row * E.N1 + c : nullptr;
+        src[u] = (i < (BM + 2) * nq && row >= 0 && row < a.M) ? gpart + (size_t)row * E.N1 + c : nullptr;
       }
       int q = 0;
       for (; q + 1 < E.P; q += 2) {
@@ -196,7 +202,7 @@
 #pragma unroll
       for (int u = 0; u < NSTG; ++u) {
         const int i = tid + 512 * u, r = i / nq, c = 4 * (i - r * nq);
-        if (i >= (CH_BM + 2) * nq) continue;
+        if (i >= (BM + 2) * nq) continue;
         float4 v = f[u];
         if (src[u]) {
           const float4 bi = gb1 ? *reinterpret_cast<const float4*>(gb1 + c) : make_float4(0.f, 0.f, 0.f, 0.f);
@@ -216,7 +222,7 @@
     __syncthreads();
     const int K0 = a_in.L[0].K16 * 16;
     const int col = wn * 32 + l31;
-    const bool cin = col < E.N2;
+    const bool cin = own && col < E.N2;
     float rs[TM][16];
 #pragma unroll
     for (int tm = 0; tm < TM; ++tm)
@@ -234,8 +240,8 @@
 #pragma unroll
     for (int tm = 0; tm < TM; ++tm)
       for (int r = 0; r < 16; ++r) acc[tm][r] = 0.f;
-    const int KSPL = (WM == 1 && 2 * E.NT2 <= WN) ? 2 : 1;
-    const bool mact = wn < E.NT2 * KSPL;
+    const int KSPL = (W == 256 && 2 * E.NT2 <= WN) ? 2 : 1;
+    const bool mact = own && wn < E.NT2 * KSPL;
     const int ect = mact ? wn % E.NT2 : 0, kp = mact ? wn / E.NT2 : 0;
     if (mact) {
       int tloc[TM];
@@ -302,7 +308,7 @@
       __syncthreads();
     }
     CTRC(2);
-    {
+    if (own) {
       const float bi = (cin && gb2) ? gb2[col] : 0.f, sc = (cin && gs2) ? gs2[col] : 1.f, sh = (cin && gh2) ? gh2[col] : 0.f;
 #pragma unroll
       for (int tm = 0; tm < TM; ++tm)
@@ -322,13 +328,13 @@
             xlo[rl * LDSW + col] = (unsigned short)lp;
           }
         }
-      have_x = true;
-    }
+    }
+    have_x = true;
     CTRC(3);
   } else
   {
     const int K0 = a_in.L[0].K16 * 16;
-    for (int i = tid; i < CH_BM * (K0 / 4); i += 512) {
+    for (int i = tid; i < BM * (K0 / 4); i += 512) {
       const int r = i / (K0 / 4), c = 4 * (i % (K0 / 4));
       float4 f = make_float4(0.f, 0.f, 0.f, 0.f);
       const int row = m0 + r;
@@ -343,7 +349,7 @@
       *reinterpret_cast<uint2*>(xlo + r * LDSW + c) = l4;
     }
   }
-  const bool full = m0 + CH_BM <= a.M;
+  const bool full = m0 + BM <= a.M;
   __syncthreads();
   CTRC(4);
 
@@ -381,29 +387,31 @@
               const int row = m0 + (wm * TM + tm) * 32 + (r & 3) + 8 * (r >> 2) + 4 * lhs;
               int orow = row;
               if (rev) {
-                const int bb = a.T >= CH_BM ? bb0 + (row >= (bb0 + 1) * a.T ? 1 : 0) : row / a.T;
-                const int tt = row - bb * a.T, Lb = a.T >= CH_BM ? (bb == bb0 ? Lb0 : Lb1) : (a.rev_len ? a.rev_len[min(bb, (a.M - 1) / a.T)] : a.T);
+                const int bb = a.T >= BM ? bb0 + (row >= (bb0 + 1) * a.T ? 1 : 0) : row / a.T;
+                const int tt = row - bb * a.T, Lb = a.T >= BM ? (bb == bb0 ? Lb0 : Lb1) : (a.rev_len ? a.rev_len[min(bb, (a.M - 1) / a.T)] : a.T);
                 orow = tt < Lb ? bb * a.T + (Lb - 1 - tt) : row;
               }
               if (row < a.M) { const float v = acc[tm][r] + bia; a.out[(size_t)orow * a.ldo + ocol] = relu_out ? fmaxf(v, 0.f) : v; }
             }
         }
       };
-      const int npass = (ngroups + 1) / 2, odd = ngroups & 1;
+      const int nmine = (ngroups - role + ROLES - 1) / ROLES;
+      const int npass = (nmine + 1) / 2, odd = nmine & 1;
       for (int ps = 0; ps < npass; ++ps) {
-        const int ng = (odd && ps == 0) ? ngroups - 1 : 2 * (ps - odd);
-        const int nt = min(ng * WN + wn, L.NT - 1), nt2 = min((ng + 1) * WN + wn, L.NT - 1);
+        const int gi = (odd && ps == 0) ? nmine - 1 : 2 * (ps - odd);
+        const int ng = role + ROLES * gi, ng2 = ng + ROLES;
+        const int nt = min(ng * WN + wn, L.NT - 1), nt2 = min(ng2 * WN + wn, L.NT - 1);
         f32x16 acc[TM], acc2[TM];
 #pragma unroll
         for (int tm = 0; tm < TM; ++tm)
           for (int r = 0; r < 16; ++r) { acc[tm][r] = 0.f; acc2[tm][r] = 0.f; }
-        if (ng + 1 < ngroups) ch_mma_loop<TM, LDSW, true, PF>(L.K16, L.NT, L.bh, L.bl, nt, L.bh, L.bl, nt2, xhi, xlo, wm * TM * 32, l31, lh, acc, acc2, krot * L.K16 >> 5);
+        if (gi + 1 < nmine) ch_mma_loop<TM, LDSW, true, PF>(L.K16, L.NT, L.bh, L.bl, nt, L.bh, L.bl, nt2, xhi, xlo, wm * TM * 32, l31, lh, acc, acc2, krot * L.K16 >> 5);
         else ch_mma_loop<TM, LDSW, false, PF>(L.K16, L.NT, L.bh, L.bl, nt, L.bh, L.bl, nt, xhi, xlo, wm * TM * 32, l31, lh, acc, acc2, krot * L.K16 >> 5);
 #ifdef TACO_TRACE
         CTRC(trci); ++trci;
 #endif
         store_group(ng, acc);
-        if (ng + 1 < ngroups) store_group(ng + 1, acc2);
+        if (gi + 1 < nmine) store_group(ng2, acc2);
 #ifdef TACO_TRACE
         CTRC(trci); ++trci;
 #endif
@@ -411,47 +419,36 @@
       continue;
     }
     const bool dual = L.type == CH_HIGHWAY;
-    if (dual && !have_x) {
+    if (dual && !have_x && own) {
 #pragma unroll
       for (int tm = 0; tm < TM; ++tm)
 #pragma unroll
         for (int r = 0; r < 16; ++r) xreg[tm][r] = a.x[(size_t)min(m0 + rloc(tm, r), a.M - 1) * a.ldx + col];
     }
     have_x = true;
-    {
-      f32x16 acc[TM], acc2[TM];
-#pragma unroll
-      for (int tm = 0; tm < TM; ++tm)
-        for (int r = 0; r < 16; ++r) { acc[tm][r] = 0.f; acc2[tm][r] = 0.f; }
-      const float bia = L.bias ? L.bias[col] : 0.f;
-      if (dual) {
-        const float bia2 = L.bias2 ? L.bias2[col] : 0.f;
-        ch_mma_loop<TM, LDSW, true, PF>(L.K16, L.NT, L.bh, L.bl, wn, L.bh2, L.bl2, wn, xhi, xlo, wm * TM * 32, l31, lh, acc, acc2, krot * L.K16 >> 5);
-#ifdef TACO_TRACE
-        CTRC(trci); ++trci;
-#endif
-#pragma unroll
-        for (int tm = 0; tm < TM; ++tm)
-#pragma unroll
-          for (int r = 0; r < 16; ++r) {
-            const float Hh = fmaxf(acc[tm][r] + bia, 0.f);
-            const float Tg = __builtin_amdgcn_rcpf(1.0f + __builtin_amdgcn_exp2f(-1.4426950408889634f * (acc2[tm][r] + bia2)));
-            xreg[tm][r] = Hh * Tg + xreg[tm][r] * (1.f - Tg);
-          }
-      } else {
-        ch_mma_loop<TM, LDSW, false, PF>(L.K16, L.NT, L.bh, L.bl, wn, L.bh, L.bl, wn, xhi, xlo, wm * TM * 32, l31, lh, acc, acc2, krot * L.K16 >> 5);
-#ifdef TACO_TRACE
-        CTRC(trci); ++trci;
-#endif
-        const bool relu = L.act == ACT_RELU;
-#pragma unroll
-        for (int tm = 0; tm < TM; ++tm)
-#pragma unroll
-          for (int r = 0; r < 16; ++r) { const float v = acc[tm][r] + bia; xreg[tm][r] = relu ? fmaxf(v, 0.f) : v; }
-      }
-    }
+    const float bia = L.bias ? L.bias[col] : 0.f, bia2 = (dual && L.bias2) ? L.bias2[col] : 0.f;
+    auto epi_highway = [&](const f32x16 (&acc)[TM], const f32x16 (&acc2)[TM]) {
+#pragma clang fp contract(off)
+#pragma unroll
+      for (int tm = 0; tm < TM; ++tm)
+#pragma unroll
+        for (int r = 0; r < 16; ++r) {
+          const float Hh = fmaxf(acc[tm][r] + bia, 0.f);
+          const float Tg = __builtin_amdgcn_rcpf(1.0f + __builtin_amdgcn_exp2f(-1.4426950408889634f * (acc2[tm][r] + bia2)));
+          const float keep = xreg[tm][r] * (1.f - Tg);
+          xreg[tm][r] = (W == 128 && r >= 14) ? Hh * Tg + keep : __builtin_fmaf(Hh, Tg, keep);
+        }
+    };
+    auto epi_dense = [&](const f32x16 (&acc)[TM]) {
+      const bool relu = L.act == ACT_RELU;
+#pragma unroll
+      for (int tm = 0; tm < TM; ++tm)
+#pragma unroll
+        for (int r = 0; r < 16; ++r) { const float v = acc[tm][r] + bia; xreg[tm][r] = relu ? fmaxf(v, 0.f) : v; }
+    };
     const bool last_hidden = (li + 1 == a.nlayers) || a_in.L[li + 1].type == CH_XPROJ;
-    if (last_hidden && a.y) {
+    auto store_y = [&]() {
+      if (!(last_hidden && a.y)) return;
 #pragma unroll
       for (int tm = 0; tm < TM; ++tm)
 #pragma unroll
@@ -459,25 +456,72 @@
           const int row = m0 + rloc(tm, r);
           if (row < a.M) a.y[(size_t)row * a.ldy + col] = xreg[tm][r];
         }
-    }
-#ifdef TACO_TRACE
-    CTRC(trci); ++trci;
-#endif
-    __syncthreads();
-#ifdef TACO_TRACE
-    CTRC(trci); ++trci;
-#endif
+    };
+    auto write_planes = [&]() {
+#pragma unroll
+      for (int tm = 0; tm < TM; ++tm)
+#pragma unroll
+        for (int r = 0; r < 16; ++r) {
+          const float f = xreg[tm][r];
+          const unsigned hp = taco_pk_bf16(f, 0.f) & 0xffffu;
+          const unsigned lp = taco_pk_bf16(f - __uint_as_float(hp << 16), 0.f) & 0xffffu;
+          xhi[rloc(tm, r) * LDSW + col] = (unsigned short)hp;
+          xlo[rloc(tm, r) * LDSW + col] = (unsigned short)lp;
+        }
+    };
+    f32x16 acc[TM], acc2[TM];
 #pragma unroll
     for (int tm = 0; tm < TM; ++tm)
-#pragma unroll
-      for (int r = 0; r < 16; ++r) {
-        const float f = xreg[tm][r];
-        const unsigned hp = taco_pk_bf16(f, 0.f) & 0xffffu;
-        const unsigned lp = taco_pk_bf16(f - __uint_as_float(hp << 16), 0.f) & 0xffffu;
-        xhi[rloc(tm, r) * LDSW + col] = (unsigned short)hp;
-        xlo[rloc(tm, r) * LDSW + col] = (unsigned short)lp;
-      }
-    __syncthreads();
+      for (int r = 0; r < 16; ++r) { acc[tm][r] = 0.f; acc2[tm][r] = 0.f; }
+    if constexpr (ROLES == 2) {
+      float* tx = reinterpret_cast<float*>(ch_smem + 2 * BM * LDSW);
+      const bool second = dual && !own;
+      if (own || dual)
+        ch_mma_loop<TM, LDSW, false, PF>(L.K16, L.NT, second ? L.bh2 : L.bh, second ? L.bl2 : L.bl, wn, second ? L.bh2 : L.bh, second ? L.bl2 : L.bl, wn,
+                                         xhi, xlo, 0, l31, lh, acc, acc2, krot * L.K16 >> 5);
+#ifdef TACO_TRACE
+      CTRC(trci); ++trci;
+#endif
+      if (second) {
+#pragma unroll
+        for (int r = 0; r < 16; ++r) tx[(wn * 16 + r) * 64 + lane] = acc[0][r];
+      }
+      __syncthreads();
+#ifdef TACO_TRACE
+      CTRC(trci); ++trci;
+#endif
+      if (own) {
+        if (dual) {
+#pragma unroll
+          for (int r = 0; r < 16; ++r) acc2[0][r] = tx[(wn * 16 + r) * 64 + lane];
+          epi_highway(acc, acc2);
+        } else epi_dense(acc);
+        store_y();
+#ifdef TACO_TRACE
+        CTRC(trci); ++trci;
+#endif
+        write_planes();
+      }
+      __syncthreads();
+    } else {
+      if (dual) ch_mma_loop<TM, LDSW, true, PF>(L.K16, L.NT, L.bh, L.bl, wn, L.bh2, L.bl2, wn, xhi, xlo, wm * TM * 32, l31, lh, acc, acc2, krot * L.K16 >> 5);
+      else ch_mma_loop<TM, LDSW, false, PF>(L.K16, L.NT, L.bh, L.bl, wn, L.bh, L.bl, wn, xhi, xlo, wm * TM * 32, l31, lh, acc, acc2, krot * L.K16 >> 5);
+#ifdef TACO_TRACE
+      CTRC(trci); ++trci;
+#endif
+      if (dual) epi_highway(acc, acc2);
+      else epi_dense(acc);
+      store_y();
+#ifdef TACO_TRACE
+      CTRC(trci); ++trci;
+#endif
+      __syncthreads();
+#ifdef TACO_TRACE
+      CTRC(trci); ++trci;
+#endif
+      write_planes();
+      __syncthreads();
+    }
 #ifdef TACO_TRACE
     CTRC(trci); ++trci;
 #endif
diff --git a/multi-speaker-tacotron-tensorflow_amd/csrc/taco_lib.hip b/multi-speaker-tacotron-tensorflow_amd/csrc/taco_lib.hip
--- a/multi-speaker-tacotron-tensorflow_amd/csrc/taco_lib.hip
+++ b/multi-speaker-tacotron-tensorflow_amd/csrc/taco_lib.hip
@@ -218,6 +218,7 @@
   unsigned* d_err = nullptr;
   int persist = 1;
   int ff_rot = 1;
+  int chain_rows = 0;
   int bf3 = 1;
   int bf3x6 = 0;
   int bf3_tn = 0;
@@ -1305,8 +1306,9 @@
   for (const ConvL& h : c.hw) if (!h.bh || !h.bh2 || h.cin != W || h.N != W) return false;
   return c.xproj.bh && c.xproj.cin == W && c.xproj.N == 6 * W;
 }
+static int chain_tile_rows(const taco_model* m, int M) { return m->chain_rows ? m->chain_rows : cdiv(M, 64) <= 128 ? 32 : 64; }
 static int run_chain(const taco_model* m, hipStream_t st, const Cbhg& c, const float* x, int in_dim, int M, int T, const int* lengths,
-                     const CbhgWs& w, const float** ff_out, const ChainEntry* entry = nullptr) {
+                     const CbhgWs& w, const float** ff_out, int bm, const ChainEntry* entry = nullptr) {
   ChainArgs a; memset(&a, 0, sizeof a);
   if (entry) a.e = *entry;
   a.x = x; a.ldx = in_dim; a.Cin = in_dim; a.out = w.xproj; a.ldo = 6 * c.rnn; a.rev_len = lengths; a.rev_col0 = 3 * c.rnn;
@@ -1321,11 +1323,12 @@
   if (c.has_dense) add(c.dense, CH_DENSE);
   for (int i = 0; i < c.depth; ++i) add(c.hw[i], CH_HIGHWAY);
   add(c.xproj, CH_XPROJ);
-  const dim3 grid(cdiv(M, CH_BM)), blk(512);
-  size_t lds = (size_t)2 * CH_BM * (c.rnn + 8) * sizeof(unsigned short);
-  if (entry) lds += (size_t)2 * (CH_BM + 2) * (entry->N1 + 8) * sizeof(unsigned short);
-  if (c.rnn == 256) hipLaunchKernelGGL((k_pointwise_chain<256>), grid, blk, lds, st, a);
-  else hipLaunchKernelGGL((k_pointwise_chain<128>), grid, blk, lds, st, a);
+  const dim3 grid(cdiv(M, bm)), blk(512);
+  const size_t lds = ch_lds_bytes(c.rnn, bm, entry ? entry->N1 : 0);
+  if (c.rnn == 256 && bm == 64) hipLaunchKernelGGL((k_pointwise_chain<256, 64>), grid, blk, lds, st, a);
+  else if (c.rnn == 256) hipLaunchKernelGGL((k_pointwise_chain<256, 32>), grid, blk, lds, st, a);
+  else if (bm == 64) hipLaunchKernelGGL((k_pointwise_chain<128, 64>), grid, blk, lds, st, a);
+  else hipLaunchKernelGGL((k_pointwise_chain<128, 32>), grid, blk, lds, st, a);
   HIPCHK(hipGetLastError());
   return 0;
 }
@@ -1400,10 +1403,11 @@
   int front_kind;
   bool entry;
   int chain_w;
+  int chain_bm;
   int launches;
   FfWhyNot why_front, why_entry, why_chain;
 };
-static FfPlan ff_plan(const taco_model* m, const Cbhg& c) {
+static FfPlan ff_plan(const taco_model* m, const Cbhg& c, int M) {
   const ConvL& P1 = c.proj[0]; const ConvL& P2 = c.proj.back();
   FfPlan p; memset(&p, 0, sizeof p);
   p.level = gemm_level(m, P1);
@@ -1415,6 +1419,7 @@
                 c.proj.size() == 2 && P2.bh && P2.kw == 3 && P2.cin == P1.N && P2.cin_pad16 == P1.N && P1.N == c.rnn && P2.N <= c.rnn && c.in_dim == P2.N
                     ? FF_WHY_NONE : FF_WHY_WIDTHS;
   p.front_kind = p.why_front ? 0 : c.front_kind; p.entry = !p.why_entry; p.chain_w = p.why_chain ? 0 : c.rnn;
+  p.chain_bm = p.chain_w ? chain_tile_rows(m, M) : 0;
   p.launches = (p.entry ? 1 : 2) + ((int)c.proj.size() - (p.entry ? 2 : 1)) + (p.chain_w ? 1 : (c.has_dense ? 1 : 0) + c.depth + 1);
   return p;
 }
@@ -1424,7 +1429,7 @@
   const int M = B * T;
   auto right = [](int k) { return k - 1 - (k - 1) / 2; };
   auto advance = [&](int win, int reach) { return win >= T ? T : std::max(0, win - reach); };
-  const FfPlan fp = ff_plan(m, c);
+  const FfPlan fp = ff_plan(m, c, M);
   const bool front = fp.front_kind && avail >= T && pg.w_bank == 0 && pg.w_p[0] == 0, entry = front && fp.entry;
   int parts = 1;
   if (front) {
@@ -1471,7 +1476,7 @@
       E.b2 = AP(m, P2.bias); E.s2 = AP(m, P2.bns); E.h2 = AP(m, P2.bnb);
       E.res = x; E.ldres = c.in_dim; E.rowvec = before_highway; E.ldrv = c.in_dim;
     }
-    TRY(run_chain(m, st, c, cur, curd, M, T, lengths, w, ff_out, entry ? &E : nullptr));
+    TRY(run_chain(m, st, c, cur, curd, M, T, lengths, w, ff_out, fp.chain_bm, entry ? &E : nullptr));
     pg.w_pt = wlast;
     return 0;
   }
@@ -1570,13 +1575,15 @@
     l.bh = v.bh; l.bl = v.bl; l.bh2 = v.bh2; l.bl2 = v.bl2; l.bias = v.bias; l.bias2 = v.bias2;
     l.type = types[i]; l.K16 = v.K16; l.NT = v.NT; l.N = v.N; l.act = ACT_RELU;
   }
-  int nwg = cdiv(M, CH_BM);
+  const int bm = chain_tile_rows(m, M);
+  int nwg = cdiv(M, bm);
   if (riders) {
     a.ntiles = nwg;
     for (int i = 0; i < 4; ++i) { a.zp[i] = riders->p[i]; a.znw[i] = riders->nw[i]; }
     nwg += std::min(192, std::max(16, 256 - nwg));
   }
-  hipLaunchKernelGGL((k_pointwise_chain<256>), dim3(nwg), dim3(512), (size_t)2 * CH_BM * (256 + 8) * sizeof(unsigned short), st, a);
+  if (bm == 64) hipLaunchKernelGGL((k_pointwise_chain<256, 64>), dim3(nwg), dim3(512), ch_lds_bytes(256, 64, 0), st, a);
+  else hipLaunchKernelGGL((k_pointwise_chain<256, 32>), dim3(nwg), dim3(512), ch_lds_bytes(256, 32, 0), st, a);
   HIPCHK(hipGetLastError());
   if (riders) register_cleared(*riders);
   return 0;
@@ -2293,10 +2300,12 @@
   HIPCHK(hipFuncSetAttribute(reinterpret_cast<const void*>(&k_bigru_rows<2, false>), hipFuncAttributeMaxDynamicSharedMemorySize, 160 * 1024));
   HIPCHK(hipFuncSetAttribute(reinterpret_cast<const void*>(&k_bigru_rows<1, true>), hipFuncAttributeMaxDynamicSharedMemorySize, 160 * 1024));
   HIPCHK(hipFuncSetAttribute(reinterpret_cast<const void*>(&k_bigru_rows<2, true>), hipFuncAttributeMaxDynamicSharedMemorySize, 160 * 1024));
-  HIPCHK(hipFuncSetAttribute(reinterpret_cast<const void*>(&k_pointwise_chain<256>), hipFuncAttributeMaxDynamicSharedMemorySize, 160 * 1024));
+  HIPCHK(hipFuncSetAttribute(reinterpret_cast<const void*>(&k_pointwise_chain<256, 64>), hipFuncAttributeMaxDynamicSharedMemorySize, 160 * 1024));
+  HIPCHK(hipFuncSetAttribute(reinterpret_cast<const void*>(&k_pointwise_chain<256, 32>), hipFuncAttributeMaxDynamicSharedMemorySize, 160 * 1024));
   HIPCHK(hipFuncSetAttribute(reinterpret_cast<const void*>(&k_head_sweep<512>), hipFuncAttributeMaxDynamicSharedMemorySize, 160 * 1024));
   HIPCHK(hipFuncSetAttribute(reinterpret_cast<const void*>(&k_head_sweep<256>), hipFuncAttributeMaxDynamicSharedMemorySize, 160 * 1024));
-  HIPCHK(hipFuncSetAttribute(reinterpret_cast<const void*>(&k_pointwise_chain<128>), hipFuncAttributeMaxDynamicSharedMemorySize, 160 * 1024));
+  HIPCHK(hipFuncSetAttribute(reinterpret_cast<const void*>(&k_pointwise_chain<128, 64>), hipFuncAttributeMaxDynamicSharedMemorySize, 160 * 1024));
+  HIPCHK(hipFuncSetAttribute(reinterpret_cast<const void*>(&k_pointwise_chain<128, 32>), hipFuncAttributeMaxDynamicSharedMemorySize, 160 * 1024));
   TRY(gemm_set_attributes());
 #define DX_ATTR(...) HIPCHK(hipFuncSetAttribute(reinterpret_cast<const void*>(&k_decoder_xcd<__VA_ARGS__>), hipFuncAttributeMaxDynamicSharedMemorySize, DX_LDS_BUDGET));
 #define PLAIN(RG, TAPE, AW, PD) DX_ATTR(RG, TAPE, false, AW, PD)
@@ -2386,6 +2395,12 @@
   m->ff_rot = on ? 0 : 1;
   return 0;
 }
+int taco_debug_set_chain_rows(taco_model* m, int rows) {
+  if (!m) return fail(TACO_ERR_ARG, "null model");
+  if (rows != 0 && rows != 32 && rows != 64) return fail(TACO_ERR_ARG, "rows is not one of 0, 32, 64");
+  m->chain_rows = rows;
+  return 0;
+}
 int taco_debug_set_att_split(taco_model* m, int slices) {
   if (!m) return fail(TACO_ERR_ARG, "null model");
   m->att_split = slices;
@@ -2510,8 +2525,8 @@
     static const char* const words[] = {"", "exact fp32 is switched on", "the six-product level has no fused kernels", "taco_debug_force_gemm_config", "a k_gemm_bf3 tile is forced"};
     return std::string(" -- no ") + kernel + ": " + (why == FF_WHY_SWITCH ? "taco_debug_set_bf3 bit " + std::to_string(bit) : why == FF_WHY_WIDTHS ? std::string(widths) : std::string(words[why]));
   };
-  auto cbhg_ff = [&](const char* name, const Cbhg& c, bool chunked) -> std::string {
-    const FfPlan fp = ff_plan(m, c);
+  auto cbhg_ff = [&](const char* name, const Cbhg& c, int M, bool chunked) -> std::string {
+    const FfPlan fp = ff_plan(m, c, M);
     const int per_layer = 1 + (int)c.proj.size() + (c.has_dense ? 1 : 0) + c.depth + 1;
     std::string r = std::string("; ") + name + " CBHG: ";
     if (m->tp) return r + launches(per_layer) + " of " + gemm_name(fp.level) + ", one per layer";
@@ -2520,7 +2535,7 @@
     r += fp.front_kind == 1 ? "k_cbhg_front<2, 80, 80, 8>" : fp.front_kind ? "k_cbhg_front<1, 144, 128, 16>" : std::string("conv bank and proj_1 on ") + gemm_name(fp.level);
     if (fp.front_kind && !fp.entry) r += " + k_front_combine";
     if (const int np = (int)c.proj.size() - (fp.entry ? 2 : 1)) r += ", " + std::to_string(np) + (np == 1 ? " projection on " : " projections on ") + gemm_name(fp.level);
-    if (fp.chain_w) r += ", k_pointwise_chain<" + std::to_string(fp.chain_w) + ">" + (fp.entry ? " (the last projection in its entry)" : "");
+    if (fp.chain_w) r += ", k_pointwise_chain<" + std::to_string(fp.chain_w) + ">" + (fp.entry ? " (the last projection in its entry)" : "") + ", " + std::to_string(fp.chain_bm) + "-row tiles";
     else r += ", " + std::to_string(fp.launches - 1 - (int)c.proj.size()) + " point-wise layers on " + gemm_name(fp.level);
     if (fp.why_front) r += ff_why("k_cbhg_front", fp.why_front, 3);
     if (fp.why_chain) r += ff_why("k_pointwise_chain", fp.why_chain, 2);
@@ -2529,9 +2544,10 @@
   };
   { const GemmLevel lv = gemm_level(m, m->linear);
     s += lv == GEMM_BF3 ? "split-bf16 MFMA, three products (k_gemm_bf3 and the fused kernels)" : lv == GEMM_BF3X6 ? "split-bf16 MFMA, six products (k_gemm_bf3<..., X6>: fp32-grade)" : "exact-fp32 MFMA (k_gemm)";
-    s += cbhg_ff("encoder", m->enc, false) + cbhg_ff("post-net", m->post, chunk != 0);
+    s += cbhg_ff("encoder", m->enc, B * T_in, false) + cbhg_ff("post-net", m->post, B * T_mel, chunk != 0);
     const FfWhyNot pw = prenet_chain_why(m);
-    if (!m->tp && !pw) s += std::string("; encoder prenet: one k_pointwise_chain launch (1 launch: embedding rows gathered, both layers") + (chunk ? ")" : "; the forward's zero fills ride in it)");
+    if (!m->tp && !pw) s += std::string("; encoder prenet: one k_pointwise_chain launch (1 launch: embedding rows gathered, both layers") + (chunk ? ")" : "; the forward's zero fills ride in it)") +
+                             ", " + std::to_string(chain_tile_rows(m, B * T_in)) + "-row tiles";
     else s += "; encoder prenet: one GEMM launch per layer (" + launches(m->hp.enc_prenet_n) + " of " + gemm_name(gemm_level(m, m->enc_prenet[0])) +
               (m->tp ? ")" : std::string(chunk ? "" : " + 1 launch of k_zero_fill_multi in front: the forward's zero fills") + ff_why("k_pointwise_chain", pw, 2) + ")");
     GemmCall g; g.ldx = 2 * m->hp.post_rnn_size; g.M = B * T_mel; g.ldo = m->hp.num_freq;
```

Result: no change. 6.453 million (median of 6 runs) (+0.7%).
